# Cheng-Lin-Li/show-attend-and-tell

Hardware: AMD Instinct MI355X
Metric: training images/sec (higher is better)
Workload: dtype bf16; 1 GPU; model=vgg16_frozen+attention_lstm512, global_batch=32, seq_len=20, vocab=5000, parallelism=dp1

## Files before the change

sat_amd/models/bptt.py:

```python

import torch

from sat_amd import _C

ACT_NONE, ACT_TANH, ACT_RELU = 0, 1, 2


def _drop(x, seed, p, salt):
    if p <= 0.0:
        return x
    return _C.hash_dropout(x, seed, p, salt)


class DecoderCoreBPTT(torch.autograd.Function):

    @staticmethod
    def forward(ctx_ag, contexts, init_memory, init_output, sentences,
                masks, emb, w1a, b1a, w1b, b1b, v, wl, bl, seed,
                p_fc, p_lstm, train_cnn, shadows=None):
        if shadows is not None:
            emb_c = shadows['emb']
            w1a_c, b1a_c = shadows['w1a'], shadows['b1a']
            w1b_c, b1b_c = shadows['w1b'], shadows['b1b']
            v_c = shadows['v'].reshape(-1)
            wl_c, bl_c = shadows['wl'], shadows['bl']
        else:
            emb_c, w1a_c, b1a_c = emb, w1a, b1a
            w1b_c, b1b_c, v_c = w1b, b1b, v
            wl_c, bl_c = wl, bl
        B, L, D = contexts.shape
        T = sentences.shape[1]
        A = w1a_c.shape[0]
        H = init_memory.shape[1]
        E = emb_c.shape[1]
        I = D + E
        dev = contexts.device

        ctx_flat = contexts.reshape(B * L, D)
        if p_fc > 0.0:
            CDROP = _C.hash_dropout_steps(ctx_flat, seed, p_fc, 0, 16, T)
            T1 = _C.dense_fwd(CDROP.reshape(T * B * L, D), w1a_c,
                              b1a_c, 1)
        else:
            CDROP = None
            T1 = _C.dense_fwd(ctx_flat, w1a_c, b1a_c, 1)

        XH = torch.empty(T * B, I + H, dtype=torch.bfloat16, device=dev)
        EXPD = torch.empty(T * B, H + D + E, dtype=torch.bfloat16,
                           device=dev)
        ODROP = torch.empty(T * B, H, dtype=torch.bfloat16, device=dev)

        t1s, t2s, tdrops, alphas = [], [], [], []
        gates_l, cprev_l = [], []

        labels_cat = sentences.t().reshape(-1)

        memory = init_memory
        state_h = init_output
        last_word = torch.zeros(B, dtype=torch.int64, device=dev)
        empty_b = _EMPTY_B(dev)
        fuse_small = (B <= 128 and (I + H) % 32 == 0
                      and (H + D + E) % 32 == 0)

        _C.hash_dropout_out(init_output, seed, p_fc, 1, ODROP[0:B])

        for t in range(T):
            s = t * 16
            sl = slice(t * B, (t + 1) * B)

            t1 = T1.reshape(-1, A)[t * B * L:(t + 1) * B * L] \
                if CDROP is not None else T1
            t2 = _C.dense_fwd(ODROP[sl], w1b_c, b1b_c, ACT_TANH)
            tdrop, att_logits = _C.attn_scores_fused(
                t1, t2, v_c, seed, p_fc, s + 2, L)
            alpha, pooled = _C.attn_pool_fwd(contexts, att_logits)

            _C.lstm_in_fuse(pooled, emb_c, last_word, state_h, seed,
                            p_lstm, s + 3, XH[sl])
            od_next = ODROP[(t + 1) * B:(t + 2) * B] if t + 1 < T \
                else empty_b
            if fuse_small:
                gates, c_new, sth_t = _C.dense_lstm_expand_fwd(
                    XH[sl], wl_c, bl_c, memory, pooled, emb_c,
                    last_word, seed, EXPD[sl], od_next,
                    1.0, p_lstm, p_fc, s)
            else:
                gates = _C.dense_fwd(XH[sl], wl_c, bl_c, ACT_NONE)
                h_raw, c_new = _C.lstm_pointwise_fwd(gates, memory, 1.0)
                out_t, sth_t = _C.expand_fuse(
                    h_raw, pooled, emb_c, last_word, seed, EXPD[sl],
                    od_next, p_lstm, p_fc, s)

            t1s.append(t1)
            t2s.append(t2)
            tdrops.append(tdrop)
            alphas.append(alpha)
            gates_l.append(gates)
            cprev_l.append(memory)

            memory = c_new
            state_h = sth_t
            last_word = labels_cat[sl]

        alpha_stack = torch.stack(alphas)
        attn_acc = (alpha_stack
                    * masks.t().reshape(T, B, 1)).sum(dim=0)

        ctx_ag.save_for_backward(
            contexts, emb_c, w1a_c, b1a_c, w1b_c, b1b_c, v_c, wl_c,
            bl_c, seed, XH, ODROP, labels_cat, masks)
        ctx_ag.leaf_mode = shadows is not None
        ctx_ag.cdrop = CDROP
        ctx_ag.saved_lists = (t1s, t2s, tdrops, alphas, gates_l, cprev_l)
        ctx_ag.dims = (B, L, D, T, A, H, E, I)
        ctx_ag.p_fc = p_fc
        ctx_ag.p_lstm = p_lstm
        ctx_ag.train_cnn = train_cnn
        return EXPD, attn_acc

    @staticmethod
    def backward(ctx_ag, d_expd, d_attn):
        (contexts, emb, w1a, b1a, w1b, b1b, v, wl, bl, seed, XH,
         ODROP, labels_cat, masks) = ctx_ag.saved_tensors
        (t1s, t2s, tdrops, alphas, gates_l,
         cprev_l) = ctx_ag.saved_lists
        B, L, D, T, A, H, E, I = ctx_ag.dims
        p_fc = ctx_ag.p_fc
        p_lstm = ctx_ag.p_lstm
        dev = contexts.device
        need_dctx = ctx_ag.train_cnn and ctx_ag.needs_input_grad[0]

        ctx_flat = contexts.reshape(B * L, D)
        if not d_expd.is_contiguous():
            d_expd = d_expd.contiguous()

        wl_t = wl.t().contiguous()
        w1b_t = w1b.t().contiguous()

        DG = torch.empty(T * B, 4 * H, dtype=torch.bfloat16, device=dev)
        DEMB = torch.empty(T * B, E, dtype=torch.bfloat16, device=dev)
        DPRE1B = torch.empty(T * B, A, dtype=torch.bfloat16, device=dev)
        DPRE1A = torch.empty(T * B * L, A, dtype=torch.bfloat16,
                             device=dev)
        CDROP = ctx_ag.cdrop

        dv_acc = torch.zeros_like(v, dtype=torch.float32)
        dctx_acc = torch.zeros_like(contexts) if need_dctx else None

        d_out_carry = torch.zeros(B, H, dtype=torch.bfloat16, device=dev)
        d_sth_carry = torch.zeros(B, H, dtype=torch.bfloat16, device=dev)
        dc_carry = torch.zeros(B, H, dtype=torch.bfloat16, device=dev)

        for t in range(T - 1, -1, -1):
            s = t * 16
            sl = slice(t * B, (t + 1) * B)
            dc_prev, dpool_dec, demb_dec = _C.dexp_lstm_bwd(
                d_expd[sl], d_out_carry, d_sth_carry, seed,
                gates_l[t], cprev_l[t], dc_carry, DG[sl],
                p_fc, p_lstm, s, D, E, 1.0)
            dgates = DG[sl]
            if B <= 128:
                dpooled, d_sth_carry = _C.dense_dx_fuse(
                    dgates, wl_t, dpool_dec, demb_dec, seed, DEMB[sl],
                    p_lstm, s + 3, D, E, H)
            else:
                dxh = _C.dense_fwd(dgates, wl_t, _EMPTY_B(dev),
                                   ACT_NONE)
                dpooled, d_sth_carry = _C.dx_fuse(
                    dxh, dpool_dec, demb_dec, seed, DEMB[sl], p_lstm,
                    s + 3, H)
            dc_carry = dc_prev

            dalpha_t = d_attn * masks[:, t].unsqueeze(1)
            dlog_att, dctx_t = _C.attn_pool_bwd(
                contexts, alphas[t], dalpha_t.contiguous(),
                dpooled, need_dctx)
            if need_dctx:
                dctx_acc += dctx_t
            sl_a = slice(t * B * L, (t + 1) * B * L)
            _dt1, dt2f, _dv = _C.attn_scores_bwd_tanh(
                tdrops[t], v, dlog_att, seed, p_fc, s + 2, L, dv_acc,
                t1s[t], DPRE1A[sl_a])

            _C.act_bwd_f32_out(dt2f, t2s[t], ACT_TANH, DPRE1B[sl])
            d_out_carry = _C.dense_fwd_drop(DPRE1B[sl], w1b_t, seed,
                                            p_fc, s + 1)

            if need_dctx:
                dcd = DPRE1A[sl_a].matmul(w1a)
                dctx_acc += _drop(dcd, seed, p_fc, s + 0) \
                    .reshape(B, L, D)

        if CDROP is not None:
            dW1a = torch.bmm(
                DPRE1A.reshape(T, B * L, A).transpose(1, 2),
                CDROP.reshape(T, B * L, D)).sum(dim=0)
        else:
            dW1a = DPRE1A.reshape(T, B * L, A).sum(0).t() \
                .matmul(ctx_flat)
        db1a = DPRE1A.sum(0, dtype=torch.float32)
        dWl = DG.t().matmul(XH)
        dbl = DG.sum(0, dtype=torch.float32)
        dW1b = DPRE1B.t().matmul(ODROP)
        db1b = DPRE1B.sum(0, dtype=torch.float32)
        demb_table = _C.embedding_bwd(
            torch.cat([torch.zeros(B, dtype=torch.int64, device=dev),
                       labels_cat[:-B]]),
            DEMB, emb.shape[0])

        d_init_output = (d_out_carry.float()
                         + d_sth_carry.float()).to(torch.bfloat16)
        d_init_memory = dc_carry

        if ctx_ag.leaf_mode:
            return (dctx_acc, d_init_memory, d_init_output, None, None,
                    demb_table.float(), dW1a.float(), db1a,
                    dW1b.float(), db1b, dv_acc.reshape(1, -1),
                    dWl.float(), dbl, None, None, None, None, None)
        bf = torch.bfloat16
        return (dctx_acc, d_init_memory, d_init_output, None, None,
                demb_table.to(bf), dW1a.to(bf), db1a.to(bf),
                dW1b.to(bf), db1b.to(bf), dv_acc.to(bf),
                dWl.to(bf), dbl.to(bf), None, None, None, None, None)


class DecodeHeadBPTT(torch.autograd.Function):

    @staticmethod
    def forward(ctx_ag, expd, wd1, bd1, wd2, bd2, sentences, masks,
                seed, p_fc, shadows=None):
        B, T = sentences.shape
        V = wd2.shape[0]
        bf = torch.bfloat16

        if shadows is not None:
            wd1c, bd1c = shadows['wd1'], shadows['bd1']
            wd2c, bd2c = shadows['wd2'], shadows['bd2']
        else:
            wd1c = wd1.to(bf)
            bd1c = bd1.to(bf)
            wd2c = wd2.to(bf)
            bd2c = bd2.to(bf)

        HID = _C.dense_fwd(expd, wd1c, bd1c, ACT_TANH)
        HD = _C.hash_dropout_slabs(HID, seed, p_fc, 7, 16, T) \
            if p_fc > 0.0 else HID
        LOGITS = _C.dense_fwd(HD, wd2c, bd2c, ACT_NONE)

        labels_cat = sentences.t().reshape(-1)
        masks_cat = masks.t().reshape(-1).contiguous()
        CE, LSE = _C.ce_fwd(LOGITS, labels_cat, masks_cat)
        ce = CE.reshape(T, B).t().contiguous()
        predictions = LOGITS.reshape(T, B, V).argmax(dim=2) \
            .t().contiguous()

        ctx_ag.save_for_backward(expd, wd1c, wd2c, HID, HD, LOGITS,
                                 LSE, labels_cat, masks_cat, seed)
        ctx_ag.T = T
        ctx_ag.p_fc = p_fc
        ctx_ag.mark_non_differentiable(predictions)
        return ce, predictions

    @staticmethod
    def backward(ctx_ag, d_ce, _d_pred):
        (expd, wd1c, wd2c, HID, HD, LOGITS, LSE, labels_cat,
         masks_cat, seed) = ctx_ag.saved_tensors
        T = ctx_ag.T
        p_fc = ctx_ag.p_fc

        dce_cat = d_ce.t().reshape(-1).contiguous().float()
        DL = _C.ce_bwd(LOGITS, labels_cat, masks_cat, LSE, dce_cat)

        fast_dx = wd2c.shape[0] % 8 == 0 and wd1c.shape[0] % 8 == 0
        if fast_dx:
            wd2_t = wd2c.t().contiguous()
            wd1_t = wd1c.t().contiguous()
            eb = torch.empty(0, dtype=torch.bfloat16, device=DL.device)
            DHD = _C.dense_fwd(DL, wd2_t, eb, 0)
        else:
            DHD = DL.matmul(wd2c)
        DHID = _C.hash_dropout_slabs(DHD, seed, p_fc, 7, 16, T) \
            if p_fc > 0.0 else DHD
        DP1 = _C.act_bwd(DHID, HID, ACT_TANH)

        if fast_dx and DL.shape[0] % 8 == 0:
            dWd2 = _C.dense_fwd(DL.t().contiguous(),
                                HD.t().contiguous(), eb, 0).float()
        else:
            dWd2 = DL.t().matmul(HD).float()
        dbd2 = DL.sum(0, dtype=torch.float32)
        dWd1 = DP1.t().matmul(expd).float()
        dbd1 = DP1.sum(0, dtype=torch.float32)
        d_expd = _C.dense_fwd(DP1, wd1_t, eb, 0) if fast_dx \
            else DP1.matmul(wd1c)

        return (d_expd, dWd1, dbd1, dWd2, dbd2, None, None, None, None,
                None)


_EMPTY = {}


def _EMPTY_B(device):
    key = str(device)
    if key not in _EMPTY:
        _EMPTY[key] = torch.empty(0, device=device, dtype=torch.bfloat16)
    return _EMPTY[key]


def run_decoder_bptt(decoder, contexts, init_memory, init_output,
                     sentences, masks):
    d = decoder
    sh = getattr(d, '_shadows', None) \
        if getattr(d, '_shadows_active', False) else None
    if sh:
        expd, attn_acc = DecoderCoreBPTT.apply(
            contexts, init_memory, init_output, sentences, masks,
            d.embedding, d.att_fc_1a.weight, d.att_fc_1a.bias,
            d.att_fc_1b.weight, d.att_fc_1b.bias, d.att_fc_2.weight,
            d.lstm_w, d.lstm_b,
            d._rng, d.nn.fc_drop_rate, d.nn.lstm_drop_rate,
            d.nn.train_cnn, sh)
        ce, predictions = DecodeHeadBPTT.apply(
            expd, d.dec_fc_1.weight, d.dec_fc_1.bias,
            d.dec_fc_2.weight, d.dec_fc_2.bias,
            sentences, masks, d._rng, d.nn.fc_drop_rate, sh)
        return ce, attn_acc, predictions
    expd, attn_acc = DecoderCoreBPTT.apply(
        contexts, init_memory, init_output, sentences, masks,
        d._emb_c, d.att_fc_1a._wc, d.att_fc_1a._bc,
        d.att_fc_1b._wc, d.att_fc_1b._bc, d._att_vc,
        d._lstm_wc, d._lstm_bc,
        d._rng, d.nn.fc_drop_rate, d.nn.lstm_drop_rate,
        d.nn.train_cnn, None)
    ce, predictions = DecodeHeadBPTT.apply(
        expd, d.dec_fc_1.weight, d.dec_fc_1.bias,
        d.dec_fc_2.weight, d.dec_fc_2.bias,
        sentences, masks, d._rng, d.nn.fc_drop_rate, None)
    return ce, attn_acc, predictions
```

sat_amd/ops/csrc/bindings.cpp:

```cpp
#include <torch/extension.h>
#include <vector>

at::Tensor dense_fwd(at::Tensor x, at::Tensor w, at::Tensor bias, int64_t act);
at::Tensor dense_fwd_drop(at::Tensor x, at::Tensor w, at::Tensor seed,
                          double p, int64_t salt);
std::vector<at::Tensor> dense_lstm_expand_fwd(
        at::Tensor xh, at::Tensor wl, at::Tensor bl, at::Tensor c_prev,
        at::Tensor pooled, at::Tensor table, at::Tensor ids,
        at::Tensor seed, at::Tensor expdrop, at::Tensor od_next,
        double fb, double p_lstm, double p_fc, int64_t s);
std::vector<at::Tensor> dexp_lstm_bwd(at::Tensor dexpd,
                                      at::Tensor d_out_carry,
                                      at::Tensor d_sth_carry,
                                      at::Tensor seed, at::Tensor gates,
                                      at::Tensor c_prev, at::Tensor dc,
                                      at::Tensor dgates_out,
                                      double p_fc, double p_lstm,
                                      int64_t s, int64_t D, int64_t E,
                                      double fb);
std::vector<at::Tensor> dense_dx_fuse(at::Tensor dgates, at::Tensor wl_t,
                                      at::Tensor dpool_dec,
                                      at::Tensor demb_dec,
                                      at::Tensor seed,
                                      at::Tensor demb_out,
                                      double p, int64_t salt,
                                      int64_t D, int64_t E, int64_t H);
at::Tensor conv3_fwd(at::Tensor input, at::Tensor weight, at::Tensor bias,
                     bool relu, bool emit_pad);
void bias_act_nhwc(at::Tensor y, at::Tensor bias, bool relu);
void scale_bias_act_nhwc(at::Tensor y, at::Tensor scale, at::Tensor shift,
                         bool relu);
at::Tensor maxpool2x2_nhwc(at::Tensor input);
at::Tensor conv_igemm_fwd(at::Tensor input, at::Tensor w_ohwi,
                          at::Tensor bias, bool relu);
at::Tensor pad1_nhwc(at::Tensor input);
at::Tensor conv_igemm_8p_fwd(at::Tensor padded, at::Tensor w_ohwi,
                             at::Tensor bias, int64_t Hh, int64_t Ww,
                             bool relu);
at::Tensor conv_igemm_glds64_fwd(at::Tensor padded, at::Tensor w_ohwi,
                                 at::Tensor bias, int64_t Hh, int64_t Ww,
                                 bool relu);
at::Tensor dense_8p_fwd(at::Tensor x, at::Tensor w, at::Tensor bias,
                        int64_t act);
at::Tensor conv3x3_wgrad(at::Tensor xpad, at::Tensor dy_rows,
                         int64_t Hh, int64_t Ww);
at::Tensor conv_igemm_glds_fwd(at::Tensor padded, at::Tensor w_ohwi,
                               at::Tensor bias, int64_t Hh, int64_t Ww,
                               bool relu);
std::vector<at::Tensor> dense_lstm_fwd(at::Tensor xh, at::Tensor wl,
                                       at::Tensor bl, at::Tensor c_prev,
                                       double fb);
std::vector<at::Tensor> lstm_pointwise_bwd_out(at::Tensor gates,
                                               at::Tensor c, at::Tensor dh,
                                               at::Tensor dc, double fb,
                                               at::Tensor dgates_out);
void lstm_in_fuse(at::Tensor pooled, at::Tensor table, at::Tensor ids,
                  at::Tensor sth, at::Tensor seed, double p, int64_t salt,
                  at::Tensor xh);
std::vector<at::Tensor> expand_fuse(at::Tensor h_raw, at::Tensor pooled,
                                    at::Tensor table, at::Tensor ids,
                                    at::Tensor seed,
                                    at::Tensor expdrop, at::Tensor od_next,
                                    double p_lstm, double p_fc, int64_t s);
std::vector<at::Tensor> dexp_fuse(at::Tensor dexpd, at::Tensor d_out_carry,
                                  at::Tensor d_sth_carry, at::Tensor seed,
                                  double p_fc, double p_lstm, int64_t s,
                                  int64_t D, int64_t E);
std::vector<at::Tensor> dx_fuse(at::Tensor dxh, at::Tensor dpool_dec,
                                at::Tensor demb_dec, at::Tensor seed,
                                at::Tensor demb_out, double p,
                                int64_t salt, int64_t H);
void hash_dropout_out(at::Tensor x, at::Tensor seed, double p,
                      int64_t salt, at::Tensor out);
at::Tensor hash_dropout_steps(at::Tensor x, at::Tensor seed, double p,
                              int64_t salt_base, int64_t salt_stride,
                              int64_t T);
void act_bwd_out(at::Tensor dy, at::Tensor y, int64_t act, at::Tensor out);
at::Tensor hash_dropout_slabs(at::Tensor x, at::Tensor seed, double p,
                              int64_t salt_base, int64_t salt_stride,
                              int64_t T);
std::vector<at::Tensor> lstm_pointwise_fwd(at::Tensor gates, at::Tensor c,
                                           double fb);
std::vector<at::Tensor> lstm_pointwise_bwd(at::Tensor gates, at::Tensor c,
                                           at::Tensor dh, at::Tensor dc,
                                           double fb);
at::Tensor act_bwd(at::Tensor dy, at::Tensor y, int64_t act);
void act_bwd_f32_out(at::Tensor dy, at::Tensor y, int64_t act,
                     at::Tensor out);
at::Tensor hash_dropout(at::Tensor x, at::Tensor seed, double p,
                        int64_t salt);
std::vector<at::Tensor> attn_pool_fwd(at::Tensor ctx, at::Tensor logits);
std::vector<at::Tensor> attn_scores_fused(at::Tensor t1, at::Tensor t2,
                                          at::Tensor v, at::Tensor seed,
                                          double p, int64_t salt, int64_t L);
std::vector<at::Tensor> attn_pool_bwd(at::Tensor ctx, at::Tensor alpha,
                                      at::Tensor dalpha, at::Tensor dpooled,
                                      bool need_dctx);
std::vector<at::Tensor> attn_scores_bwd(at::Tensor tdrop, at::Tensor v,
                                        at::Tensor dlogits, at::Tensor seed,
                                        double p, int64_t salt, int64_t L);
std::vector<at::Tensor> attn_scores_bwd_acc(at::Tensor tdrop, at::Tensor v,
                                            at::Tensor dlogits,
                                            at::Tensor seed, double p,
                                            int64_t salt, int64_t L,
                                            at::Tensor dv_acc);
std::vector<at::Tensor> attn_scores_bwd_tanh(
        at::Tensor tdrop, at::Tensor v, at::Tensor dlogits,
        at::Tensor seed, double p, int64_t salt, int64_t L,
        at::Tensor dv_acc, at::Tensor t1y, at::Tensor dt1_out);
at::Tensor embedding_fwd(at::Tensor ids, at::Tensor table);
at::Tensor embedding_bwd(at::Tensor ids, at::Tensor dy, int64_t rows);
std::vector<at::Tensor> ce_fwd(at::Tensor logits, at::Tensor labels,
                               at::Tensor mask);
at::Tensor ce_bwd(at::Tensor logits, at::Tensor labels, at::Tensor mask,
                  at::Tensor lse, at::Tensor dloss);
at::Tensor grad_sq_norm(std::vector<at::Tensor> grads);
at::Tensor sq_norm_mt(at::Tensor desc, at::Tensor cum, int64_t n_tensors,
                      int64_t total);
void adam_step_mt(at::Tensor desc, at::Tensor cum, int64_t n_tensors,
                  int64_t total, at::Tensor step_dev, double lr0,
                  double decay_factor, double steps_per_decay, double b1,
                  double b2, double eps, double clip, at::Tensor gsq,
                  bool zero_grads, bool vec4);
void adam_step(std::vector<at::Tensor> params, std::vector<at::Tensor> grads,
               std::vector<at::Tensor> ms, std::vector<at::Tensor> vs,
               at::Tensor step_dev, double lr0, double decay_factor,
               double steps_per_decay, double b1, double b2, double eps,
               double clip, at::Tensor gsq);

PYBIND11_MODULE(TORCH_EXTENSION_NAME, m) {
    m.def("dense_fwd", &dense_fwd, "MFMA GEMM + bias/act (bf16)");
    m.def("dense_fwd_drop", &dense_fwd_drop,
          "skinny GEMM with hash-dropout fused into the split-K epilogue");
    m.def("dense_lstm_expand_fwd", &dense_lstm_expand_fwd,
          "gates GEMM + LSTM gate math + expand scatter in 2 launches");
    m.def("dexp_lstm_bwd", &dexp_lstm_bwd,
          "dexp scatter + LSTM pointwise backward in one launch");
    m.def("dense_dx_fuse", &dense_dx_fuse,
          "dxh GEMM with the dx scatter fused into the epilogue");
    m.def("bias_act_nhwc", &bias_act_nhwc);
    m.def("scale_bias_act_nhwc", &scale_bias_act_nhwc);
    m.def("maxpool2x2_nhwc", &maxpool2x2_nhwc);
    m.def("conv_igemm_fwd", &conv_igemm_fwd);
    m.def("pad1_nhwc", &pad1_nhwc);
    m.def("conv_igemm_glds_fwd", &conv_igemm_glds_fwd);
    m.def("conv_igemm_8p_fwd", &conv_igemm_8p_fwd,
          "8-phase deep-pipelined implicit-GEMM conv (Cout%256==0)");
    m.def("conv_igemm_glds64_fwd", &conv_igemm_glds64_fwd);
    m.def("dense_8p_fwd", &dense_8p_fwd,
          "8-phase deep-pipelined dense GEMM (big-M shapes)");
    m.def("conv3x3_wgrad", &conv3x3_wgrad,
          "3x3 conv weight grad: transpose-staged MFMA split-K reduce");
    m.def("dense_lstm_fwd", &dense_lstm_fwd);
    m.def("conv3_fwd", &conv3_fwd,
          "direct NHWC conv for 3-channel 3x3/s1 (VGG conv1_1)");
    m.def("lstm_pointwise_bwd_out", &lstm_pointwise_bwd_out);
    m.def("lstm_in_fuse", &lstm_in_fuse);
    m.def("expand_fuse", &expand_fuse);
    m.def("dexp_fuse", &dexp_fuse);
    m.def("dx_fuse", &dx_fuse);
    m.def("hash_dropout_out", &hash_dropout_out);
    m.def("hash_dropout_steps", &hash_dropout_steps);
    m.def("act_bwd_out", &act_bwd_out);
    m.def("hash_dropout_slabs", &hash_dropout_slabs);
    m.def("lstm_pointwise_fwd", &lstm_pointwise_fwd);
    m.def("lstm_pointwise_bwd", &lstm_pointwise_bwd);
    m.def("act_bwd", &act_bwd);
    m.def("act_bwd_f32_out", &act_bwd_f32_out);
    m.def("hash_dropout", &hash_dropout);
    m.def("attn_pool_fwd", &attn_pool_fwd);
    m.def("attn_scores_fused", &attn_scores_fused);
    m.def("attn_pool_bwd", &attn_pool_bwd);
    m.def("attn_scores_bwd", &attn_scores_bwd);
    m.def("attn_scores_bwd_acc", &attn_scores_bwd_acc);
    m.def("attn_scores_bwd_tanh", &attn_scores_bwd_tanh,
          "scores backward with fused tanh-bwd dt1 into a given slab");
    m.def("embedding_fwd", &embedding_fwd);
    m.def("embedding_bwd", &embedding_bwd);
    m.def("ce_fwd", &ce_fwd);
    m.def("ce_bwd", &ce_bwd);
    m.def("grad_sq_norm", &grad_sq_norm);
    m.def("sq_norm_mt", &sq_norm_mt);
    m.def("adam_step_mt", &adam_step_mt);
    m.def("adam_step", &adam_step);
}
```

sat_amd/ops/csrc/bptt_fuse.hip:

```cpp

#include "common.h"


__global__ void lstm_in_fuse_kernel(const bf16* __restrict__ pooled,
                                    const bf16* __restrict__ table,
                                    const int64_t* __restrict__ ids,
                                    const bf16* __restrict__ sth,
                                    const int64_t* __restrict__ seed_p,
                                    bf16* __restrict__ xh,
                                    int B, int D, int E, int H,
                                    float p, int salt) {
    const uint32_t seed = (uint32_t)(*seed_p);
    const int I = D + E;
    const int W = I + H;
    int64_t idx = (int64_t)blockIdx.x * blockDim.x + threadIdx.x;
    if (idx >= (int64_t)B * W) return;
    int b = idx / W, j = idx % W;
    float val;
    if (j < I) {
        val = (j < D) ? bf2f(pooled[(int64_t)b * D + j])
                      : bf2f(table[ids[b] * E + (j - D)]);
        val *= drop_scale(seed, salt, (uint32_t)(b * I + j), p);
    } else {
        val = bf2f(sth[(int64_t)b * H + (j - I)]);
    }
    xh[idx] = f2bf(val);
}

void lstm_in_fuse(at::Tensor pooled, at::Tensor table, at::Tensor ids,
                  at::Tensor sth, at::Tensor seed, double p, int64_t salt,
                  at::Tensor xh) {
    int B = pooled.size(0), D = pooled.size(1), E = table.size(1),
        H = sth.size(1);
    int64_t n = (int64_t)B * (D + E + H);
    hipStream_t s = at::cuda::getCurrentCUDAStream();
    hipLaunchKernelGGL(lstm_in_fuse_kernel, dim3(cdiv(n, 256)), dim3(256),
                       0, s,
                       (const bf16*)pooled.data_ptr(),
                       (const bf16*)table.data_ptr(),
                       (const int64_t*)ids.data_ptr(),
                       (const bf16*)sth.data_ptr(),
                       (const int64_t*)seed.data_ptr(),
                       (bf16*)xh.data_ptr(), B, D, E, H,
                       (float)p, (int)salt);
    HIP_OK(hipGetLastError());
}


__global__ void expand_fuse_kernel(const bf16* __restrict__ h_raw,
                                   const bf16* __restrict__ pooled,
                                   const bf16* __restrict__ table,
                                   const int64_t* __restrict__ ids,
                                   const int64_t* __restrict__ seed_p,
                                   bf16* __restrict__ out_t,
                                   bf16* __restrict__ sth_t,
                                   bf16* __restrict__ expdrop,
                                   bf16* __restrict__ od_next,
                                   int B, int H, int D, int E,
                                   float p_lstm, float p_fc, int s) {
    const uint32_t seed = (uint32_t)(*seed_p);
    const int W = H + D + E;
    int64_t idx = (int64_t)blockIdx.x * blockDim.x + threadIdx.x;
    if (idx >= (int64_t)B * W) return;
    int b = idx / W, j = idx % W;
    float val;
    if (j < H) {
        float h = bf2f(h_raw[(int64_t)b * H + j]);
        uint32_t hidx = (uint32_t)(b * H + j);
        float ot = h * drop_scale(seed, s + 4, hidx, p_lstm);
        out_t[(int64_t)b * H + j] = f2bf(ot);
        sth_t[(int64_t)b * H + j] =
            f2bf(h * drop_scale(seed, s + 5, hidx, p_lstm));
        if (od_next != nullptr)
            od_next[(int64_t)b * H + j] =
                f2bf(ot * drop_scale(seed, s + 16 + 1, hidx, p_fc));
        val = ot;
    } else if (j < H + D) {
        val = bf2f(pooled[(int64_t)b * D + (j - H)]);
    } else {
        val = bf2f(table[ids[b] * E + (j - H - D)]);
    }
    expdrop[idx] = f2bf(val * drop_scale(seed, s + 6,
                                         (uint32_t)(b * W + j), p_fc));
}

std::vector<at::Tensor> expand_fuse(at::Tensor h_raw, at::Tensor pooled,
                                    at::Tensor table, at::Tensor ids,
                                    at::Tensor seed,
                                    at::Tensor expdrop, at::Tensor od_next,
                                    double p_lstm, double p_fc,
                                    int64_t s) {
    int B = h_raw.size(0), H = h_raw.size(1), D = pooled.size(1),
        E = table.size(1);
    auto out_t = at::empty_like(h_raw);
    auto sth_t = at::empty_like(h_raw);
    bf16* od_ptr = nullptr;
    if (od_next.defined() && od_next.numel() > 0)
        od_ptr = (bf16*)od_next.data_ptr();
    int64_t n = (int64_t)B * (H + D + E);
    hipStream_t st = at::cuda::getCurrentCUDAStream();
    hipLaunchKernelGGL(expand_fuse_kernel, dim3(cdiv(n, 256)), dim3(256),
                       0, st,
                       (const bf16*)h_raw.data_ptr(),
                       (const bf16*)pooled.data_ptr(),
                       (const bf16*)table.data_ptr(),
                       (const int64_t*)ids.data_ptr(),
                       (const int64_t*)seed.data_ptr(),
                       (bf16*)out_t.data_ptr(), (bf16*)sth_t.data_ptr(),
                       (bf16*)expdrop.data_ptr(), od_ptr,
                       B, H, D, E, (float)p_lstm, (float)p_fc, (int)s);
    HIP_OK(hipGetLastError());
    return {out_t, sth_t};
}


__global__ void dexp_fuse_kernel(const bf16* __restrict__ dexpd,
                                 const bf16* __restrict__ d_out_carry,
                                 const bf16* __restrict__ d_sth_carry,
                                 const int64_t* __restrict__ seed_p,
                                 bf16* __restrict__ dh_raw,
                                 bf16* __restrict__ dpool_dec,
                                 bf16* __restrict__ demb_dec,
                                 int B, int H, int D, int E,
                                 float p_fc, float p_lstm, int s) {
    const uint32_t seed = (uint32_t)(*seed_p);
    const int W = H + D + E;
    int64_t idx = (int64_t)blockIdx.x * blockDim.x + threadIdx.x;
    if (idx >= (int64_t)B * W) return;
    int b = idx / W, j = idx % W;
    float dexp = bf2f(dexpd[idx])
        * drop_scale(seed, s + 6, (uint32_t)(b * W + j), p_fc);
    if (j < H) {
        uint32_t hidx = (uint32_t)(b * H + j);
        float dout = dexp + bf2f(d_out_carry[(int64_t)b * H + j]);
        float dh = dout * drop_scale(seed, s + 4, hidx, p_lstm)
            + bf2f(d_sth_carry[(int64_t)b * H + j])
            * drop_scale(seed, s + 5, hidx, p_lstm);
        dh_raw[(int64_t)b * H + j] = f2bf(dh);
    } else if (j < H + D) {
        dpool_dec[(int64_t)b * D + (j - H)] = f2bf(dexp);
    } else {
        demb_dec[(int64_t)b * E + (j - H - D)] = f2bf(dexp);
    }
}

std::vector<at::Tensor> dexp_fuse(at::Tensor dexpd, at::Tensor d_out_carry,
                                  at::Tensor d_sth_carry, at::Tensor seed,
                                  double p_fc, double p_lstm, int64_t s,
                                  int64_t D, int64_t E) {
    int B = d_out_carry.size(0), H = d_out_carry.size(1);
    auto dh_raw = at::empty_like(d_out_carry);
    auto dpool = at::empty({B, D}, d_out_carry.options());
    auto demb = at::empty({B, E}, d_out_carry.options());
    int64_t n = (int64_t)B * (H + D + E);
    hipStream_t st = at::cuda::getCurrentCUDAStream();
    hipLaunchKernelGGL(dexp_fuse_kernel, dim3(cdiv(n, 256)), dim3(256),
                       0, st,
                       (const bf16*)dexpd.data_ptr(),
                       (const bf16*)d_out_carry.data_ptr(),
                       (const bf16*)d_sth_carry.data_ptr(),
                       (const int64_t*)seed.data_ptr(),
                       (bf16*)dh_raw.data_ptr(), (bf16*)dpool.data_ptr(),
                       (bf16*)demb.data_ptr(), B, H, (int)D, (int)E,
                       (float)p_fc, (float)p_lstm, (int)s);
    HIP_OK(hipGetLastError());
    return {dh_raw, dpool, demb};
}


__global__ void dx_fuse_kernel(const bf16* __restrict__ dxh,
                               const bf16* __restrict__ dpool_dec,
                               const bf16* __restrict__ demb_dec,
                               const int64_t* __restrict__ seed_p,
                               bf16* __restrict__ dpooled,
                               bf16* __restrict__ demb_out,
                               bf16* __restrict__ dsth,
                               int B, int D, int E, int H,
                               float p, int salt) {
    const uint32_t seed = (uint32_t)(*seed_p);
    const int I = D + E;
    const int W = I + H;
    int64_t idx = (int64_t)blockIdx.x * blockDim.x + threadIdx.x;
    if (idx >= (int64_t)B * W) return;
    int b = idx / W, j = idx % W;
    float g = bf2f(dxh[idx]);
    if (j < I) {
        g *= drop_scale(seed, salt, (uint32_t)(b * I + j), p);
        if (j < D)
            dpooled[(int64_t)b * D + j] =
                f2bf(g + bf2f(dpool_dec[(int64_t)b * D + j]));
        else
            demb_out[(int64_t)b * E + (j - D)] =
                f2bf(g + bf2f(demb_dec[(int64_t)b * E + (j - D)]));
    } else {
        dsth[(int64_t)b * H + (j - I)] = f2bf(g);
    }
}

std::vector<at::Tensor> dx_fuse(at::Tensor dxh, at::Tensor dpool_dec,
                                at::Tensor demb_dec, at::Tensor seed,
                                at::Tensor demb_out, double p,
                                int64_t salt, int64_t H) {
    int B = dpool_dec.size(0), D = dpool_dec.size(1), E = demb_dec.size(1);
    auto dpooled = at::empty_like(dpool_dec);
    auto dsth = at::empty({B, H}, dpool_dec.options());
    int64_t n = (int64_t)B * (D + E + H);
    hipStream_t st = at::cuda::getCurrentCUDAStream();
    hipLaunchKernelGGL(dx_fuse_kernel, dim3(cdiv(n, 256)), dim3(256),
                       0, st,
                       (const bf16*)dxh.data_ptr(),
                       (const bf16*)dpool_dec.data_ptr(),
                       (const bf16*)demb_dec.data_ptr(),
                       (const int64_t*)seed.data_ptr(),
                       (bf16*)dpooled.data_ptr(),
                       (bf16*)demb_out.data_ptr(),
                       (bf16*)dsth.data_ptr(),
                       B, D, E, (int)H, (float)p, (int)salt);
    HIP_OK(hipGetLastError());
    return {dpooled, dsth};
}


__global__ void hash_dropout_out_kernel(const bf16* __restrict__ x,
                                        const int64_t* __restrict__ seed_p,
                                        bf16* __restrict__ y,
                                        int64_t n, float p, int salt) {
    const uint32_t seed = (uint32_t)(*seed_p);
    int64_t idx = (int64_t)blockIdx.x * blockDim.x + threadIdx.x;
    if (idx >= n) return;
    y[idx] = f2bf(bf2f(x[idx])
                  * drop_scale(seed, salt, (uint32_t)idx, p));
}

void hash_dropout_out(at::Tensor x, at::Tensor seed, double p,
                      int64_t salt, at::Tensor out) {
    int64_t n = x.numel();
    hipStream_t s = at::cuda::getCurrentCUDAStream();
    hipLaunchKernelGGL(hash_dropout_out_kernel, dim3(cdiv(n, 256)),
                       dim3(256), 0, s,
                       (const bf16*)x.data_ptr(),
                       (const int64_t*)seed.data_ptr(),
                       (bf16*)out.data_ptr(), n, (float)p, (int)salt);
    HIP_OK(hipGetLastError());
}


__global__ void hash_dropout_steps_kernel(const bf16* __restrict__ x,
                                          const int64_t* __restrict__ seed_p,
                                          bf16* __restrict__ y,
                                          int64_t n, int T, float p,
                                          int salt_base, int salt_stride) {
    const uint32_t seed = (uint32_t)(*seed_p);
    int64_t i8 = ((int64_t)blockIdx.x * blockDim.x + threadIdx.x) * 8;
    int64_t total = n * T;
    int64_t stride = (int64_t)gridDim.x * blockDim.x * 8;
    for (; i8 < total; i8 += stride) {
        int t = (int)(i8 / n);
        int64_t j = i8 % n;
        int salt = salt_base + t * salt_stride;
        bf16x8 v = *(const bf16x8*)(x + j);
        bf16x8 o;
#pragma unroll
        for (int e = 0; e < 8; ++e)
            o[e] = f2bf(bf2f(v[e]) * drop_scale(seed, salt,
                                                (uint32_t)(j + e), p));
        *(bf16x8*)(y + i8) = o;
    }
}

at::Tensor hash_dropout_steps(at::Tensor x, at::Tensor seed, double p,
                              int64_t salt_base, int64_t salt_stride,
                              int64_t T) {
    int64_t n = x.numel();
    TORCH_CHECK(n % 8 == 0, "hash_dropout_steps needs numel % 8 == 0");
    auto y = at::empty({T, x.size(0), x.size(1)}, x.options());
    hipStream_t s = at::cuda::getCurrentCUDAStream();
    int blocks = (int)std::min<int64_t>(cdiv(n * T, 256 * 8), 16384);
    hipLaunchKernelGGL(hash_dropout_steps_kernel, dim3(blocks), dim3(256),
                       0, s,
                       (const bf16*)x.data_ptr(),
                       (const int64_t*)seed.data_ptr(),
                       (bf16*)y.data_ptr(), n, (int)T, (float)p,
                       (int)salt_base, (int)salt_stride);
    HIP_OK(hipGetLastError());
    return y;
}

__global__ void act_bwd_out_kernel(const bf16* __restrict__ dy,
                                   const bf16* __restrict__ y,
                                   bf16* __restrict__ dpre,
                                   int64_t n, int act) {
    int64_t idx = (int64_t)blockIdx.x * blockDim.x + threadIdx.x;
    if (idx >= n) return;
    float g = bf2f(dy[idx]);
    float yv = bf2f(y[idx]);
    if (act == 1) g *= (1.f - yv * yv);
    else if (act == 2) g *= (yv > 0.f ? 1.f : 0.f);
    dpre[idx] = f2bf(g);
}

void act_bwd_out(at::Tensor dy, at::Tensor y, int64_t act, at::Tensor out) {
    int64_t n = dy.numel();
    hipStream_t s = at::cuda::getCurrentCUDAStream();
    hipLaunchKernelGGL(act_bwd_out_kernel, dim3(cdiv(n, 256)), dim3(256),
                       0, s,
                       (const bf16*)dy.data_ptr(), (const bf16*)y.data_ptr(),
                       (bf16*)out.data_ptr(), n, (int)act);
    HIP_OK(hipGetLastError());
}

__global__ void act_bwd_f32_out_kernel(const float* __restrict__ dy,
                                       const bf16* __restrict__ y,
                                       bf16* __restrict__ dpre,
                                       int64_t n, int act) {
    int64_t idx = (int64_t)blockIdx.x * blockDim.x + threadIdx.x;
    if (idx >= n) return;
    float g = dy[idx];
    float yv = bf2f(y[idx]);
    if (act == 1) g *= (1.f - yv * yv);
    else if (act == 2) g *= (yv > 0.f ? 1.f : 0.f);
    dpre[idx] = f2bf(g);
}

void act_bwd_f32_out(at::Tensor dy, at::Tensor y, int64_t act,
                     at::Tensor out) {
    int64_t n = dy.numel();
    hipStream_t s = at::cuda::getCurrentCUDAStream();
    hipLaunchKernelGGL(act_bwd_f32_out_kernel, dim3(cdiv(n, 256)),
                       dim3(256), 0, s,
                       (const float*)dy.data_ptr(),
                       (const bf16*)y.data_ptr(),
                       (bf16*)out.data_ptr(), n, (int)act);
    HIP_OK(hipGetLastError());
}


__global__ void hash_dropout_slabs_kernel(const bf16* __restrict__ x,
                                          const int64_t* __restrict__ seed_p,
                                          bf16* __restrict__ y,
                                          int64_t slab_elems, int T,
                                          float p, int salt_base,
                                          int salt_stride) {
    const uint32_t seed = (uint32_t)(*seed_p);
    int64_t i8 = ((int64_t)blockIdx.x * blockDim.x + threadIdx.x) * 8;
    int64_t total = slab_elems * T;
    if (i8 >= total) return;
    int t = (int)(i8 / slab_elems);
    int64_t j = i8 % slab_elems;
    int salt = salt_base + t * salt_stride;
    bf16x8 v = *(const bf16x8*)(x + i8);
    bf16x8 o;
#pragma unroll
    for (int e = 0; e < 8; ++e)
        o[e] = f2bf(bf2f(v[e])
                    * drop_scale(seed, salt, (uint32_t)(j + e), p));
    *(bf16x8*)(y + i8) = o;
}

at::Tensor hash_dropout_slabs(at::Tensor x, at::Tensor seed, double p,
                              int64_t salt_base, int64_t salt_stride,
                              int64_t T) {
    if (p <= 0.0) return x;
    int64_t n = x.numel();
    int64_t slab = n / T;
    TORCH_CHECK(slab % 8 == 0 && n % T == 0);
    auto y = at::empty_like(x);
    hipStream_t s = at::cuda::getCurrentCUDAStream();
    hipLaunchKernelGGL(hash_dropout_slabs_kernel,
                       dim3(cdiv(n / 8, 256)), dim3(256), 0, s,
                       (const bf16*)x.data_ptr(),
                       (const int64_t*)seed.data_ptr(),
                       (bf16*)y.data_ptr(), slab, (int)T, (float)p,
                       (int)salt_base, (int)salt_stride);
    HIP_OK(hipGetLastError());
    return y;
}


__global__ void dexp_lstm_bwd_kernel(const bf16* __restrict__ dexpd,
                                     const bf16* __restrict__ d_out_carry,
                                     const bf16* __restrict__ d_sth_carry,
                                     const int64_t* __restrict__ seed_p,
                                     const bf16* __restrict__ gates,
                                     const bf16* __restrict__ c,
                                     const bf16* __restrict__ dc,
                                     bf16* __restrict__ dgates,
                                     bf16* __restrict__ dc_prev,
                                     bf16* __restrict__ dpool_dec,
                                     bf16* __restrict__ demb_dec,
                                     int B, int H, int D, int E,
                                     float p_fc, float p_lstm, int s,
                                     float fb) {
    const uint32_t seed = (uint32_t)(*seed_p);
    const int W = H + D + E;
    int64_t idx = (int64_t)blockIdx.x * blockDim.x + threadIdx.x;
    if (idx >= (int64_t)B * W) return;
    int b = idx / W, j = idx % W;
    float dexp = bf2f(dexpd[idx])
        * drop_scale(seed, s + 6, (uint32_t)(b * W + j), p_fc);
    if (j < H) {
        uint32_t hidx = (uint32_t)(b * H + j);
        float dout = dexp + bf2f(d_out_carry[(int64_t)b * H + j]);
        float dhv = dout * drop_scale(seed, s + 4, hidx, p_lstm)
            + bf2f(d_sth_carry[(int64_t)b * H + j])
            * drop_scale(seed, s + 5, hidx, p_lstm);
        const bf16* gp = gates + (int64_t)b * 4 * H + j;
        float g[4], dg[4], dcp;
#pragma unroll
        for (int q = 0; q < 4; ++q) g[q] = bf2f(gp[q * H]);
        float dcv = (dc != nullptr) ? bf2f(dc[(int64_t)b * H + j]) : 0.f;
        lstm_cell_bwd(g, bf2f(c[(int64_t)b * H + j]), dhv, dcv, fb, dg,
                      dcp);
        bf16* dgp = dgates + (int64_t)b * 4 * H + j;
#pragma unroll
        for (int q = 0; q < 4; ++q) dgp[q * H] = f2bf(dg[q]);
        dc_prev[(int64_t)b * H + j] = f2bf(dcp);
    } else if (j < H + D) {
        dpool_dec[(int64_t)b * D + (j - H)] = f2bf(dexp);
    } else {
        demb_dec[(int64_t)b * E + (j - H - D)] = f2bf(dexp);
    }
}

std::vector<at::Tensor> dexp_lstm_bwd(at::Tensor dexpd,
                                      at::Tensor d_out_carry,
                                      at::Tensor d_sth_carry,
                                      at::Tensor seed, at::Tensor gates,
                                      at::Tensor c_prev, at::Tensor dc,
                                      at::Tensor dgates_out,
                                      double p_fc, double p_lstm,
                                      int64_t s, int64_t D, int64_t E,
                                      double fb) {
    CHECK_GPU(dexpd); CHECK_BF16(dexpd);
    int B = d_out_carry.size(0), H = d_out_carry.size(1);
    TORCH_CHECK(dexpd.numel() == (int64_t)B * (H + D + E));
    TORCH_CHECK(dgates_out.numel() == (int64_t)B * 4 * H);
    auto dc_prev = at::empty({B, H}, dexpd.options());
    auto dpool_dec = at::empty({B, D}, dexpd.options());
    auto demb_dec = at::empty({B, E}, dexpd.options());
    const bf16* dc_ptr = nullptr;
    if (dc.defined() && dc.numel() > 0)
        dc_ptr = (const bf16*)dc.data_ptr();
    int64_t n = (int64_t)B * (H + D + E);
    hipStream_t st = at::cuda::getCurrentCUDAStream();
    hipLaunchKernelGGL(dexp_lstm_bwd_kernel, dim3(cdiv(n, 256)),
                       dim3(256), 0, st,
                       (const bf16*)dexpd.data_ptr(),
                       (const bf16*)d_out_carry.data_ptr(),
                       (const bf16*)d_sth_carry.data_ptr(),
                       (const int64_t*)seed.data_ptr(),
                       (const bf16*)gates.data_ptr(),
                       (const bf16*)c_prev.data_ptr(), dc_ptr,
                       (bf16*)dgates_out.data_ptr(),
                       (bf16*)dc_prev.data_ptr(),
                       (bf16*)dpool_dec.data_ptr(),
                       (bf16*)demb_dec.data_ptr(),
                       B, H, (int)D, (int)E,
                       (float)p_fc, (float)p_lstm, (int)s, (float)fb);
    HIP_OK(hipGetLastError());
    return {dc_prev, dpool_dec, demb_dec};
}
```

sat_amd/ops/csrc/gemm.hip:

```cpp

#include "common.h"

at::Tensor dense_8p_fwd(at::Tensor x, at::Tensor w, at::Tensor bias,
                        int64_t act);
at::Tensor hash_dropout(at::Tensor x, at::Tensor seed, double p,
                        int64_t salt);

#define BK 64
#define LDS_STRIDE (BK + 8)

#define ACT_NONE 0
#define ACT_TANH 1
#define ACT_RELU 2

__device__ __forceinline__ float apply_act(float v, int act) {
    if (act == ACT_TANH) return tanhf(v);
    if (act == ACT_RELU) return fmaxf(v, 0.f);
    return v;
}


template <int WR, int WC, int FM, int FN>
__global__ __launch_bounds__(256)
void tiled_gemm_kernel(const bf16* __restrict__ A,
                       const bf16* __restrict__ W,
                       const bf16* __restrict__ bias,
                       bf16* __restrict__ Y,
                       int M, int N, int K, int act,
                       float* __restrict__ Yf, int kchunk) {
    constexpr int BM = WR * FM * 16;
    constexpr int BN = WC * FN * 16;
    __shared__ bf16 As[BM * LDS_STRIDE];
    __shared__ bf16 Bs[BN * LDS_STRIDE];

    const int tid = threadIdx.x;
    const int lane = tid & 63;
    const int wave = tid >> 6;
    const int wr = wave / WC;
    const int wc = wave % WC;

    const int bm = blockIdx.y * BM;
    const int bn = blockIdx.x * BN;

    floatx4 acc[FM][FN];
#pragma unroll
    for (int i = 0; i < FM; ++i)
#pragma unroll
        for (int j = 0; j < FN; ++j)
            acc[i][j] = floatx4{0.f, 0.f, 0.f, 0.f};

    const int lrow = lane & 15;
    const int kgrp = lane >> 4;

    constexpr int A_CHUNKS = BM * BK / 8 / 256;
    constexpr int B_CHUNKS = BN * BK / 8 / 256;

    int kbeg = 0, kend = K;
    if (Yf != nullptr) {
        kbeg = blockIdx.z * kchunk;
        kend = min(K, kbeg + kchunk);
    }
    for (int k0 = kbeg; k0 < kend; k0 += BK) {
#pragma unroll
        for (int i = 0; i < A_CHUNKS; ++i) {
            int q = tid + 256 * i;
            int row = q >> 3;
            int c8 = (q & 7) * 8;
            int gk = k0 + c8;
            bf16x8 v = {};
            int ga = bm + row;
            if (ga < M && gk + 8 <= K) {
                v = *(const bf16x8*)(A + (int64_t)ga * K + gk);
            } else if (ga < M) {
                for (int e = 0; e < 8; ++e)
                    if (gk + e < K) v[e] = A[(int64_t)ga * K + gk + e];
            }
            *(bf16x8*)(As + row * LDS_STRIDE + c8) = v;
        }
#pragma unroll
        for (int i = 0; i < B_CHUNKS; ++i) {
            int q = tid + 256 * i;
            int row = q >> 3;
            int c8 = (q & 7) * 8;
            int gk = k0 + c8;
            bf16x8 v = {};
            int gb = bn + row;
            if (gb < N && gk + 8 <= K) {
                v = *(const bf16x8*)(W + (int64_t)gb * K + gk);
            } else if (gb < N) {
                for (int e = 0; e < 8; ++e)
                    if (gk + e < K) v[e] = W[(int64_t)gb * K + gk + e];
            }
            *(bf16x8*)(Bs + row * LDS_STRIDE + c8) = v;
        }
        __syncthreads();

#pragma unroll
        for (int kk = 0; kk < BK / 32; ++kk) {
            bf16x8 a_frag[FM], b_frag[FN];
            const int kof = kk * 32 + kgrp * 8;
#pragma unroll
            for (int mi = 0; mi < FM; ++mi)
                a_frag[mi] = *(const bf16x8*)(
                    As + (wr * FM * 16 + mi * 16 + lrow) * LDS_STRIDE + kof);
#pragma unroll
            for (int ni = 0; ni < FN; ++ni)
                b_frag[ni] = *(const bf16x8*)(
                    Bs + (wc * FN * 16 + ni * 16 + lrow) * LDS_STRIDE + kof);
#pragma unroll
            for (int mi = 0; mi < FM; ++mi)
#pragma unroll
                for (int ni = 0; ni < FN; ++ni)
                    acc[mi][ni] = __builtin_amdgcn_mfma_f32_16x16x32_bf16(
                        a_frag[mi], b_frag[ni], acc[mi][ni], 0, 0, 0);
        }
        __syncthreads();
    }

    float* slab = (Yf != nullptr)
        ? Yf + (int64_t)blockIdx.z * M * N : nullptr;
#pragma unroll
    for (int ni = 0; ni < FN; ++ni) {
        int col = bn + wc * FN * 16 + ni * 16 + (lane & 15);
        float bv = (bias != nullptr && col < N) ? bf2f(bias[col]) : 0.f;
#pragma unroll
        for (int mi = 0; mi < FM; ++mi) {
#pragma unroll
            for (int r = 0; r < 4; ++r) {
                int row = bm + wr * FM * 16 + mi * 16 + (lane >> 4) * 4 + r;
                if (row < M && col < N) {
                    if (slab != nullptr)
                        slab[(int64_t)row * N + col] = acc[mi][ni][r];
                    else
                        Y[(int64_t)row * N + col] =
                            f2bf(apply_act(acc[mi][ni][r] + bv, act));
                }
            }
        }
    }
}


template <int RF>
__global__ __launch_bounds__(256)
void skinny_gemm_kernel(const bf16* __restrict__ A,
                        const bf16* __restrict__ W,
                        const bf16* __restrict__ bias,
                        bf16* __restrict__ Y,
                        float* __restrict__ Yf,
                        int M, int N, int K, int act, int splitk) {
    const int lane = threadIdx.x & 63;
    const int wave = threadIdx.x >> 6;
    const int n0 = blockIdx.x * 64 + wave * 16;
    const bool active = (n0 < N);

    const int kq = blockIdx.y;
    const int kchunk = ((K / 32 + splitk - 1) / splitk) * 32;
    const int kbeg = kq * kchunk;
    const int kend = min(K, kbeg + kchunk);

    const int lrow = lane & 15;
    const int kgrp = lane >> 4;

    floatx4 acc[RF];
#pragma unroll
    for (int i = 0; i < RF; ++i)
        acc[i] = floatx4{0.f, 0.f, 0.f, 0.f};

    const bool wfull = (n0 + 16 <= N);
    if (active) {
        for (int k = kbeg; k < kend; k += 32) {
            const int kof = k + kgrp * 8;
            bf16x8 b_frag = {};
            if (kof + 8 <= K) {
                int gb = n0 + lrow;
                if (wfull || gb < N)
                    b_frag = *(const bf16x8*)(W + (int64_t)gb * K + kof);
            } else if (kof < K) {
                int gb = n0 + lrow;
                if (wfull || gb < N)
                    for (int e = 0; e < 8 && kof + e < K; ++e)
                        b_frag[e] = W[(int64_t)gb * K + kof + e];
            }
#pragma unroll
            for (int mi = 0; mi < RF; ++mi) {
                bf16x8 a0 = {};
                int ar = mi * 16 + lrow;
                if (kof + 8 <= K) {
                    if (ar < M)
                        a0 = *(const bf16x8*)(A + (int64_t)ar * K + kof);
                } else if (kof < K) {
                    if (ar < M)
                        for (int e = 0; e < 8 && kof + e < K; ++e)
                            a0[e] = A[(int64_t)ar * K + kof + e];
                }
                acc[mi] = __builtin_amdgcn_mfma_f32_16x16x32_bf16(
                    a0, b_frag, acc[mi], 0, 0, 0);
            }
        }
    }

    const int col = n0 + (lane & 15);
    if (!active || col >= N) return;
    if (Yf == nullptr) {
        float bv = (bias != nullptr) ? bf2f(bias[col]) : 0.f;
#pragma unroll
        for (int mi = 0; mi < RF; ++mi)
#pragma unroll
            for (int r = 0; r < 4; ++r) {
                int row = mi * 16 + (lane >> 4) * 4 + r;
                if (row < M)
                    Y[(int64_t)row * N + col] =
                        f2bf(apply_act(acc[mi][r] + bv, act));
            }
        return;
    }

    float* slab = Yf + (int64_t)kq * M * N;
#pragma unroll
    for (int mi = 0; mi < RF; ++mi)
#pragma unroll
        for (int r = 0; r < 4; ++r) {
            int row = mi * 16 + (lane >> 4) * 4 + r;
            if (row < M)
                slab[(int64_t)row * N + col] = acc[mi][r];
        }
}

__global__ void skinny_epilogue_kernel(const float* __restrict__ Yf,
                                       const bf16* __restrict__ bias,
                                       bf16* __restrict__ Y,
                                       int64_t n, int N, int act,
                                       int splitk) {
    int64_t idx = (int64_t)blockIdx.x * blockDim.x + threadIdx.x;
    if (idx >= n) return;
    float v = sum_slabs(Yf, n, idx, splitk);
    if (bias != nullptr) v += bf2f(bias[idx % N]);
    Y[idx] = f2bf(apply_act(v, act));
}

__global__ void dense_glds_kernel(const bf16* __restrict__ A,
                                  const bf16* __restrict__ W,
                                  const bf16* __restrict__ bias,
                                  bf16* __restrict__ Y,
                                  int M, int N, int K, int act);


static bool is_skinny(int64_t M, int64_t K) {
    return M <= 128 && K % 32 == 0;
}

struct SkinnyPlan { int nblocks, splitk; };

static SkinnyPlan skinny_plan(int64_t N, int64_t K) {
    int nblocks = cdiv(N, 64);
    int splitk = 1;
    while (nblocks * splitk < 192 && splitk < 8 &&
           (int)(K / 32) >= 2 * splitk)
        splitk *= 2;
    return {nblocks, splitk};
}

static void launch_skinny(hipStream_t stream, const at::Tensor& x,
                          const at::Tensor& w, const bf16* bias, bf16* y,
                          float* yf, int act, SkinnyPlan plan) {
    const int M = x.size(0), K = x.size(1), N = w.size(0);
    TORCH_CHECK(is_skinny(M, K),
                "skinny GEMM: M <= 128 and K % 32 == 0 only");
    auto kernel = M <= 32 ? skinny_gemm_kernel<2>
                : M <= 64 ? skinny_gemm_kernel<4>
                          : skinny_gemm_kernel<8>;
    hipLaunchKernelGGL(kernel, dim3(plan.nblocks, plan.splitk), dim3(256),
                       0, stream, (const bf16*)x.data_ptr(),
                       (const bf16*)w.data_ptr(), bias, y, yf, M, N, K,
                       act, plan.splitk);
}

static at::Tensor skinny_slabs(hipStream_t stream, const at::Tensor& x,
                               const at::Tensor& w) {
    SkinnyPlan plan = skinny_plan(w.size(0), x.size(1));
    auto yf = at::empty({plan.splitk, x.size(0), w.size(0)},
                        x.options().dtype(at::kFloat));
    launch_skinny(stream, x, w, nullptr, nullptr, (float*)yf.data_ptr(),
                  ACT_NONE, plan);
    return yf;
}

static void launch_tiled(hipStream_t stream, const at::Tensor& x,
                         const at::Tensor& w, const bf16* bias, bf16* y,
                         float* yf, int act, int splitk, int kchunk) {
    const int M = x.size(0), K = x.size(1), N = w.size(0);
    const bool narrow = N <= 512;
    auto kernel = narrow ? tiled_gemm_kernel<4, 1, 2, 4>
                         : tiled_gemm_kernel<2, 2, 4, 4>;
    dim3 grid(cdiv(N, narrow ? 64 : 128), cdiv(M, 128), splitk);
    hipLaunchKernelGGL(kernel, grid, dim3(256), 0, stream,
                       (const bf16*)x.data_ptr(),
                       (const bf16*)w.data_ptr(), bias, y, M, N, K, act,
                       yf, kchunk);
}

static void launch_epilogue(hipStream_t stream, const at::Tensor& yf,
                            const bf16* bias, at::Tensor& y, int act) {
    int64_t n = y.numel();
    hipLaunchKernelGGL(skinny_epilogue_kernel, dim3(cdiv(n, 256)),
                       dim3(256), 0, stream, (const float*)yf.data_ptr(),
                       bias, (bf16*)y.data_ptr(), n, (int)y.size(1), act,
                       (int)yf.size(0));
}

at::Tensor dense_fwd(at::Tensor x, at::Tensor w, at::Tensor bias,
                     int64_t act) {
    CHECK_GPU(x); CHECK_CONTIG(x); CHECK_BF16(x);
    CHECK_GPU(w); CHECK_CONTIG(w); CHECK_BF16(w);
    TORCH_CHECK(x.dim() == 2 && w.dim() == 2, "dense_fwd expects 2-D inputs");
    const int64_t M = x.size(0), K = x.size(1), N = w.size(0);
    TORCH_CHECK(w.size(1) == K, "weight inner dim mismatch");
    TORCH_CHECK(K % 8 == 0, "K must be a multiple of 8 (bf16x8 loads)");
    const bf16* bias_ptr = nullptr;
    if (bias.defined() && bias.numel() > 0) {
        CHECK_GPU(bias); CHECK_CONTIG(bias); CHECK_BF16(bias);
        TORCH_CHECK(bias.numel() == N, "bias size mismatch");
        bias_ptr = (const bf16*)bias.data_ptr();
    }
    const bool skinny = is_skinny(M, K);
    if (!skinny && M >= 16384 && N >= 256 && N % 8 == 0 && K % 64 == 0
        && K >= 128) {
        return dense_8p_fwd(x, w, bias_ptr != nullptr ? bias : at::Tensor(),
                            act);
    }
    auto y = at::empty({M, N}, x.options());
    hipStream_t stream = at::cuda::getCurrentCUDAStream();

    if (skinny) {
        SkinnyPlan plan = skinny_plan(N, K);
        if (plan.splitk == 1) {
            launch_skinny(stream, x, w, bias_ptr, (bf16*)y.data_ptr(),
                          nullptr, (int)act, plan);
        } else {
            auto yf = skinny_slabs(stream, x, w);
            launch_epilogue(stream, yf, bias_ptr, y, (int)act);
        }
    } else if (M >= 16384 && N % 128 == 0 && K % 64 == 0) {
        dim3 grid(cdiv(N, 128), cdiv(M, 128));
        hipLaunchKernelGGL(dense_glds_kernel, grid, dim3(256), 0,
                           stream,
                           (const bf16*)x.data_ptr(),
                           (const bf16*)w.data_ptr(), bias_ptr,
                           (bf16*)y.data_ptr(), (int)M, (int)N, (int)K,
                           (int)act);
    } else {
        int tiles = cdiv(N, N <= 512 ? 64 : 128) * cdiv(M, 128);
        int splitk = 1;
        while (tiles * splitk < 160 && splitk < 8
               && K >= 128 * 2 * splitk)
            splitk *= 2;
        int kchunk = cdiv(cdiv(K, splitk), 64) * 64;
        splitk = cdiv(K, kchunk);
        if (splitk == 1) {
            launch_tiled(stream, x, w, bias_ptr, (bf16*)y.data_ptr(),
                         nullptr, (int)act, 1, kchunk);
        } else {
            auto yf = at::empty({splitk, M, N},
                                x.options().dtype(at::kFloat));
            launch_tiled(stream, x, w, bias_ptr, (bf16*)y.data_ptr(),
                         (float*)yf.data_ptr(), (int)act, splitk, kchunk);
            launch_epilogue(stream, yf, bias_ptr, y, (int)act);
        }
    }
    HIP_OK(hipGetLastError());
    return y;
}


__global__ void skinny_epilogue_drop_kernel(
        const float* __restrict__ Yf, bf16* __restrict__ Y,
        const int64_t* __restrict__ seed_p, int64_t n, int splitk,
        float p, int salt) {
    int64_t idx = (int64_t)blockIdx.x * blockDim.x + threadIdx.x;
    if (idx >= n) return;
    float v = sum_slabs(Yf, n, idx, splitk);
    v *= drop_scale((uint32_t)(*seed_p), salt, (uint32_t)idx, p);
    Y[idx] = f2bf(v);
}

at::Tensor dense_fwd_drop(at::Tensor x, at::Tensor w, at::Tensor seed,
                          double p, int64_t salt) {
    CHECK_GPU(x); CHECK_CONTIG(x); CHECK_BF16(x);
    CHECK_GPU(w); CHECK_CONTIG(w); CHECK_BF16(w);
    int64_t M = x.size(0), K = x.size(1), N = w.size(0);
    if (p <= 0.0 || !is_skinny(M, K)) {
        auto y = dense_fwd(x, w, at::Tensor(), ACT_NONE);
        return p > 0.0 ? hash_dropout(y, seed, p, salt) : y;
    }
    auto y = at::empty({M, N}, x.options());
    hipStream_t stream = at::cuda::getCurrentCUDAStream();
    auto yf = skinny_slabs(stream, x, w);
    int64_t n = M * N;
    hipLaunchKernelGGL(skinny_epilogue_drop_kernel,
                       dim3(cdiv(n, 256)), dim3(256), 0, stream,
                       (const float*)yf.data_ptr(), (bf16*)y.data_ptr(),
                       (const int64_t*)seed.data_ptr(), n,
                       (int)yf.size(0), (float)p, (int)salt);
    HIP_OK(hipGetLastError());
    return y;
}


__device__ __forceinline__ void sum_gates(const float* __restrict__ Yf,
                                          const bf16* __restrict__ bias,
                                          bf16* __restrict__ gates,
                                          int B, int H, int b, int hh,
                                          int splitk, float g[4]) {
    int64_t n = (int64_t)B * 4 * H;
#pragma unroll
    for (int q = 0; q < 4; ++q) {
        int64_t off = (int64_t)b * 4 * H + q * H + hh;
        float acc = sum_slabs(Yf, n, off, splitk);
        if (bias != nullptr) acc += bf2f(bias[q * H + hh]);
        gates[off] = f2bf(acc);
        g[q] = acc;
    }
}

__global__ void skinny_epi_lstm_kernel(const float* __restrict__ Yf,
                                       const bf16* __restrict__ bias,
                                       const bf16* __restrict__ c_prev,
                                       bf16* __restrict__ gates,
                                       bf16* __restrict__ h_out,
                                       bf16* __restrict__ c_out,
                                       int B, int H, int splitk,
                                       float fb) {
    int idx = blockIdx.x * blockDim.x + threadIdx.x;
    if (idx >= B * H) return;
    float g[4], cn, h;
    sum_gates(Yf, bias, gates, B, H, idx / H, idx % H, splitk, g);
    lstm_cell_fwd(g, bf2f(c_prev[idx]), fb, cn, h);
    h_out[idx] = f2bf(h);
    c_out[idx] = f2bf(cn);
}

std::vector<at::Tensor> dense_lstm_fwd(at::Tensor xh, at::Tensor wl,
                                       at::Tensor bl, at::Tensor c_prev,
                                       double fb) {
    int64_t M = xh.size(0), N = wl.size(0);
    int B = c_prev.size(0), H = c_prev.size(1);
    TORCH_CHECK(M == B && N == 4 * H);
    auto gates = at::empty({M, N}, xh.options());
    auto h_out = at::empty_like(c_prev);
    auto c_out = at::empty_like(c_prev);
    hipStream_t s = at::cuda::getCurrentCUDAStream();
    auto yf = skinny_slabs(s, xh, wl);
    hipLaunchKernelGGL(skinny_epi_lstm_kernel,
                       dim3(cdiv(B * H, 256)), dim3(256), 0, s,
                       (const float*)yf.data_ptr(),
                       (const bf16*)bl.data_ptr(),
                       (const bf16*)c_prev.data_ptr(),
                       (bf16*)gates.data_ptr(), (bf16*)h_out.data_ptr(),
                       (bf16*)c_out.data_ptr(), B, H, (int)yf.size(0),
                       (float)fb);
    HIP_OK(hipGetLastError());
    return {gates, h_out, c_out};
}



__global__ __launch_bounds__(256)
void dense_glds_kernel(const bf16* __restrict__ A,
                       const bf16* __restrict__ W,
                       const bf16* __restrict__ bias,
                       bf16* __restrict__ Y,
                       int M, int N, int K, int act) {
    constexpr int BM = 128, BN = 128, BKc = 64;
    __shared__ bf16 lds[2 * BM * BKc];
    bf16* As = lds;
    bf16* Bs = lds + BM * BKc;

    const int tid = threadIdx.x;
    const int lane = tid & 63;
    const int wave = tid >> 6;
    const int wr = wave >> 1, wc = wave & 1;
    const int bm = blockIdx.y * BM;
    const int bn = blockIdx.x * BN;

    const bf16* aSrc[4];
    const bf16* wSrc[4];
    const int ci8 = (lane & 7) * 8;
#pragma unroll
    for (int i = 0; i < 4; ++i) {
        int r = wave * 32 + i * 8 + (lane >> 3);
        int swz = (r & 4) ? 16 : 0;
        int ga = bm + r;
        if (ga >= M) ga = M - 1;
        aSrc[i] = A + (int64_t)ga * K + (ci8 ^ swz);
        int gb = bn + r;
        if (gb >= N) gb = N - 1;
        wSrc[i] = W + (int64_t)gb * K + (ci8 ^ swz);
    }

    floatx4 acc[4][4];
#pragma unroll
    for (int i = 0; i < 4; ++i)
#pragma unroll
        for (int j = 0; j < 4; ++j)
            acc[i][j] = floatx4{0.f, 0.f, 0.f, 0.f};

    const int lrow = lane & 15;
    const int kgrp = lane >> 4;

    for (int k0 = 0; k0 < K; k0 += BKc) {
#pragma unroll
        for (int i = 0; i < 4; ++i) {
            __builtin_amdgcn_global_load_lds(
                (const __attribute__((address_space(1))) uint32_t*)
                    (aSrc[i] + k0),
                (__attribute__((address_space(3))) uint32_t*)
                    (As + (wave * 32 + i * 8) * BKc),
                16, 0, 0);
            __builtin_amdgcn_global_load_lds(
                (const __attribute__((address_space(1))) uint32_t*)
                    (wSrc[i] + k0),
                (__attribute__((address_space(3))) uint32_t*)
                    (Bs + (wave * 32 + i * 8) * BKc),
                16, 0, 0);
        }
        __syncthreads();

#pragma unroll
        for (int kk = 0; kk < 2; ++kk) {
            bf16x8 a_frag[4], b_frag[4];
            const int kof = kk * 32 + kgrp * 8;
#pragma unroll
            for (int mi = 0; mi < 4; ++mi) {
                int r = wr * 64 + mi * 16 + lrow;
                a_frag[mi] = *(const bf16x8*)(
                    As + r * BKc + (kof ^ ((r & 4) ? 16 : 0)));
            }
#pragma unroll
            for (int ni = 0; ni < 4; ++ni) {
                int r = wc * 64 + ni * 16 + lrow;
                b_frag[ni] = *(const bf16x8*)(
                    Bs + r * BKc + (kof ^ ((r & 4) ? 16 : 0)));
            }
#pragma unroll
            for (int mi = 0; mi < 4; ++mi)
#pragma unroll
                for (int ni = 0; ni < 4; ++ni)
                    acc[mi][ni] = __builtin_amdgcn_mfma_f32_16x16x32_bf16(
                        a_frag[mi], b_frag[ni], acc[mi][ni], 0, 0, 0);
        }
        __syncthreads();
    }

#pragma unroll
    for (int ni = 0; ni < 4; ++ni) {
        int col = bn + wc * 64 + ni * 16 + (lane & 15);
        float bv = (bias != nullptr && col < N) ? bf2f(bias[col]) : 0.f;
#pragma unroll
        for (int mi = 0; mi < 4; ++mi) {
#pragma unroll
            for (int r = 0; r < 4; ++r) {
                int row = bm + wr * 64 + mi * 16 + (lane >> 4) * 4 + r;
                if (row < M && col < N) {
                    float vv = acc[mi][ni][r] + bv;
                    Y[(int64_t)row * N + col] = f2bf(apply_act(vv, act));
                }
            }
        }
    }
}


__global__ void skinny_epi_dx_kernel(const float* __restrict__ Yf,
                                     const bf16* __restrict__ dpool_dec,
                                     const bf16* __restrict__ demb_dec,
                                     const int64_t* __restrict__ seed_p,
                                     bf16* __restrict__ dpooled,
                                     bf16* __restrict__ demb_out,
                                     bf16* __restrict__ dsth,
                                     int64_t n, int splitk,
                                     int B, int D, int E, int H,
                                     float p, int salt) {
    const uint32_t seed = (uint32_t)(*seed_p);
    const int I = D + E;
    const int W = I + H;
    int64_t idx = (int64_t)blockIdx.x * blockDim.x + threadIdx.x;
    if (idx >= n) return;
    float g = sum_slabs(Yf, n, idx, splitk);
    int b = (int)(idx / W), j = (int)(idx % W);
    if (j < I) {
        g *= drop_scale(seed, salt, (uint32_t)(b * I + j), p);
        if (j < D)
            dpooled[(int64_t)b * D + j] =
                f2bf(g + bf2f(dpool_dec[(int64_t)b * D + j]));
        else
            demb_out[(int64_t)b * E + (j - D)] =
                f2bf(g + bf2f(demb_dec[(int64_t)b * E + (j - D)]));
    } else {
        dsth[(int64_t)b * H + (j - I)] = f2bf(g);
    }
}

std::vector<at::Tensor> dense_dx_fuse(at::Tensor dgates, at::Tensor wl_t,
                                      at::Tensor dpool_dec,
                                      at::Tensor demb_dec,
                                      at::Tensor seed,
                                      at::Tensor demb_out,
                                      double p, int64_t salt,
                                      int64_t D, int64_t E, int64_t H) {
    CHECK_GPU(dgates); CHECK_CONTIG(dgates); CHECK_BF16(dgates);
    CHECK_GPU(wl_t); CHECK_CONTIG(wl_t); CHECK_BF16(wl_t);
    int64_t M = dgates.size(0), N = wl_t.size(0);
    TORCH_CHECK(N == D + E + H);
    auto dpooled = at::empty({M, D}, dgates.options());
    auto dsth = at::empty({M, H}, dgates.options());
    hipStream_t stream = at::cuda::getCurrentCUDAStream();
    auto yf = skinny_slabs(stream, dgates, wl_t);
    int64_t n = M * N;
    hipLaunchKernelGGL(skinny_epi_dx_kernel, dim3(cdiv(n, 256)),
                       dim3(256), 0, stream,
                       (const float*)yf.data_ptr(),
                       (const bf16*)dpool_dec.data_ptr(),
                       (const bf16*)demb_dec.data_ptr(),
                       (const int64_t*)seed.data_ptr(),
                       (bf16*)dpooled.data_ptr(),
                       (bf16*)demb_out.data_ptr(),
                       (bf16*)dsth.data_ptr(),
                       n, (int)yf.size(0), (int)M, (int)D, (int)E, (int)H,
                       (float)p, (int)salt);
    HIP_OK(hipGetLastError());
    return {dpooled, dsth};
}


__global__ void skinny_epi_lstm_expand_kernel(
        const float* __restrict__ Yf, const bf16* __restrict__ bias,
        const bf16* __restrict__ c_prev,
        const bf16* __restrict__ pooled,
        const bf16* __restrict__ table,
        const int64_t* __restrict__ ids,
        const int64_t* __restrict__ seed_p,
        bf16* __restrict__ gates, bf16* __restrict__ c_out,
        bf16* __restrict__ sth_t, bf16* __restrict__ expdrop,
        bf16* __restrict__ od_next,
        int B, int H, int D, int E, int splitk,
        float fb, float p_lstm, float p_fc, int s) {
    const uint32_t seed = (uint32_t)(*seed_p);
    const int W = H + D + E;
    int64_t idx = (int64_t)blockIdx.x * blockDim.x + threadIdx.x;
    if (idx >= (int64_t)B * W) return;
    int b = idx / W, j = idx % W;
    float val;
    if (j < H) {
        float g[4], cn, h;
        sum_gates(Yf, bias, gates, B, H, b, j, splitk, g);
        lstm_cell_fwd(g, bf2f(c_prev[(int64_t)b * H + j]), fb, cn, h);
        c_out[(int64_t)b * H + j] = f2bf(cn);
        uint32_t hidx = (uint32_t)(b * H + j);
        float ot = h * drop_scale(seed, s + 4, hidx, p_lstm);
        sth_t[(int64_t)b * H + j] =
            f2bf(h * drop_scale(seed, s + 5, hidx, p_lstm));
        if (od_next != nullptr)
            od_next[(int64_t)b * H + j] =
                f2bf(ot * drop_scale(seed, s + 16 + 1, hidx, p_fc));
        val = ot;
    } else if (j < H + D) {
        val = bf2f(pooled[(int64_t)b * D + (j - H)]);
    } else {
        val = bf2f(table[ids[b] * E + (j - H - D)]);
    }
    expdrop[idx] = f2bf(val * drop_scale(seed, s + 6,
                                         (uint32_t)(b * W + j), p_fc));
}

std::vector<at::Tensor> dense_lstm_expand_fwd(
        at::Tensor xh, at::Tensor wl, at::Tensor bl, at::Tensor c_prev,
        at::Tensor pooled, at::Tensor table, at::Tensor ids,
        at::Tensor seed, at::Tensor expdrop, at::Tensor od_next,
        double fb, double p_lstm, double p_fc, int64_t s) {
    int64_t M = xh.size(0), N = wl.size(0);
    int B = c_prev.size(0), H = c_prev.size(1);
    int D = pooled.size(1), E = table.size(1);
    TORCH_CHECK(M == B && N == 4 * H);
    auto gates = at::empty({M, N}, xh.options());
    auto c_out = at::empty({B, H}, xh.options());
    auto sth_t = at::empty({B, H}, xh.options());
    hipStream_t stream = at::cuda::getCurrentCUDAStream();
    auto yf = skinny_slabs(stream, xh, wl);
    const bf16* bias_ptr = nullptr;
    if (bl.defined() && bl.numel() > 0)
        bias_ptr = (const bf16*)bl.data_ptr();
    bf16* od_ptr = nullptr;
    if (od_next.defined() && od_next.numel() > 0)
        od_ptr = (bf16*)od_next.data_ptr();
    int64_t n = (int64_t)B * (H + D + E);
    hipLaunchKernelGGL(skinny_epi_lstm_expand_kernel,
                       dim3(cdiv(n, 256)), dim3(256), 0, stream,
                       (const float*)yf.data_ptr(), bias_ptr,
                       (const bf16*)c_prev.data_ptr(),
                       (const bf16*)pooled.data_ptr(),
                       (const bf16*)table.data_ptr(),
                       (const int64_t*)ids.data_ptr(),
                       (const int64_t*)seed.data_ptr(),
                       (bf16*)gates.data_ptr(),
                       (bf16*)c_out.data_ptr(),
                       (bf16*)sth_t.data_ptr(),
                       (bf16*)expdrop.data_ptr(), od_ptr,
                       B, H, D, E, (int)yf.size(0),
                       (float)fb, (float)p_lstm, (float)p_fc, (int)s);
    HIP_OK(hipGetLastError());
    return {gates, c_out, sth_t};
}
```

sat_amd/ops/csrc/kernels.hip:

```cpp

#include "common.h"


__global__ void lstm_pw_fwd_kernel(const bf16* __restrict__ gates,
                                   const bf16* __restrict__ c,
                                   bf16* __restrict__ h_out,
                                   bf16* __restrict__ c_out,
                                   int B, int H, float fb) {
    int idx = blockIdx.x * blockDim.x + threadIdx.x;
    if (idx >= B * H) return;
    int b = idx / H, hh = idx % H;
    const bf16* gp = gates + (int64_t)b * 4 * H + hh;
    float g[4];
#pragma unroll
    for (int q = 0; q < 4; ++q) g[q] = bf2f(gp[q * H]);
    float cn, h;
    lstm_cell_fwd(g, bf2f(c[idx]), fb, cn, h);
    h_out[idx] = f2bf(h);
    c_out[idx] = f2bf(cn);
}

__global__ void lstm_pw_bwd_kernel(const bf16* __restrict__ gates,
                                   const bf16* __restrict__ c,
                                   const bf16* __restrict__ dh,
                                   const bf16* __restrict__ dc,
                                   bf16* __restrict__ dgates,
                                   bf16* __restrict__ dc_prev,
                                   int B, int H, float fb) {
    int idx = blockIdx.x * blockDim.x + threadIdx.x;
    if (idx >= B * H) return;
    int b = idx / H, hh = idx % H;
    const bf16* gp = gates + (int64_t)b * 4 * H + hh;
    float g[4], dg[4], dcp;
#pragma unroll
    for (int q = 0; q < 4; ++q) g[q] = bf2f(gp[q * H]);
    float dcv = (dc != nullptr) ? bf2f(dc[idx]) : 0.f;
    lstm_cell_bwd(g, bf2f(c[idx]), bf2f(dh[idx]), dcv, fb, dg, dcp);
    bf16* dgp = dgates + (int64_t)b * 4 * H + hh;
#pragma unroll
    for (int q = 0; q < 4; ++q) dgp[q * H] = f2bf(dg[q]);
    dc_prev[idx] = f2bf(dcp);
}

std::vector<at::Tensor> lstm_pointwise_fwd(at::Tensor gates, at::Tensor c,
                                           double fb) {
    CHECK_GPU(gates); CHECK_CONTIG(gates); CHECK_BF16(gates);
    CHECK_GPU(c); CHECK_CONTIG(c); CHECK_BF16(c);
    int B = c.size(0), H = c.size(1);
    TORCH_CHECK(gates.size(0) == B && gates.size(1) == 4 * H);
    auto h_out = at::empty_like(c);
    auto c_out = at::empty_like(c);
    int n = B * H;
    hipStream_t s = at::cuda::getCurrentCUDAStream();
    hipLaunchKernelGGL(lstm_pw_fwd_kernel, dim3(cdiv(n, 256)), dim3(256), 0, s,
                       (const bf16*)gates.data_ptr(), (const bf16*)c.data_ptr(),
                       (bf16*)h_out.data_ptr(), (bf16*)c_out.data_ptr(),
                       B, H, (float)fb);
    HIP_OK(hipGetLastError());
    return {h_out, c_out};
}

std::vector<at::Tensor> lstm_pointwise_bwd_out(at::Tensor gates,
                                               at::Tensor c, at::Tensor dh,
                                               at::Tensor dc, double fb,
                                               at::Tensor dgates_out) {
    CHECK_GPU(gates); CHECK_CONTIG(gates); CHECK_BF16(gates);
    int B = c.size(0), H = c.size(1);
    at::Tensor dgates;
    if (dgates_out.defined() && dgates_out.numel() > 0)
        dgates = dgates_out;
    else
        dgates = at::empty_like(gates);
    auto dc_prev = at::empty_like(c);
    const bf16* dc_ptr = nullptr;
    if (dc.defined() && dc.numel() > 0) dc_ptr = (const bf16*)dc.data_ptr();
    int n = B * H;
    hipStream_t s = at::cuda::getCurrentCUDAStream();
    hipLaunchKernelGGL(lstm_pw_bwd_kernel, dim3(cdiv(n, 256)), dim3(256), 0, s,
                       (const bf16*)gates.data_ptr(), (const bf16*)c.data_ptr(),
                       (const bf16*)dh.data_ptr(), dc_ptr,
                       (bf16*)dgates.data_ptr(), (bf16*)dc_prev.data_ptr(),
                       B, H, (float)fb);
    HIP_OK(hipGetLastError());
    return {dgates, dc_prev};
}

std::vector<at::Tensor> lstm_pointwise_bwd(at::Tensor gates, at::Tensor c,
                                           at::Tensor dh, at::Tensor dc,
                                           double fb) {
    return lstm_pointwise_bwd_out(gates, c, dh, dc, fb, at::Tensor());
}


__global__ void act_bwd_kernel(const bf16* __restrict__ dy,
                               const bf16* __restrict__ y,
                               bf16* __restrict__ dpre,
                               int64_t n, int act) {
    int64_t idx = (int64_t)blockIdx.x * blockDim.x + threadIdx.x;
    if (idx >= n) return;
    float g = bf2f(dy[idx]);
    float yv = bf2f(y[idx]);
    if (act == 1) g *= (1.f - yv * yv);
    else if (act == 2) g *= (yv > 0.f ? 1.f : 0.f);
    dpre[idx] = f2bf(g);
}

at::Tensor act_bwd(at::Tensor dy, at::Tensor y, int64_t act) {
    CHECK_GPU(dy); CHECK_CONTIG(dy); CHECK_BF16(dy);
    CHECK_GPU(y); CHECK_CONTIG(y); CHECK_BF16(y);
    auto dpre = at::empty_like(dy);
    int64_t n = dy.numel();
    hipStream_t s = at::cuda::getCurrentCUDAStream();
    hipLaunchKernelGGL(act_bwd_kernel, dim3(cdiv(n, 256)), dim3(256), 0, s,
                       (const bf16*)dy.data_ptr(), (const bf16*)y.data_ptr(),
                       (bf16*)dpre.data_ptr(), n, (int)act);
    HIP_OK(hipGetLastError());
    return dpre;
}


#define MAX_L 1024


__global__ void hash_dropout_kernel(const bf16* __restrict__ x,
                                    const int64_t* __restrict__ seed_p,
                                    bf16* __restrict__ y,
                                    int64_t n, float p, int salt) {
    const uint32_t seed = (uint32_t)(*seed_p);
    int64_t idx = (int64_t)blockIdx.x * blockDim.x + threadIdx.x;
    int64_t stride = (int64_t)gridDim.x * blockDim.x;
    for (int64_t i = idx * 8; i < n; i += stride * 8) {
        if (i + 8 <= n) {
            bf16x8 v = *(const bf16x8*)(x + i);
            bf16x8 o;
#pragma unroll
            for (int e = 0; e < 8; ++e)
                o[e] = f2bf(bf2f(v[e]) *
                            drop_scale(seed, salt, (uint32_t)(i + e), p));
            *(bf16x8*)(y + i) = o;
        } else {
            for (int64_t j = i; j < n; ++j)
                y[j] = f2bf(bf2f(x[j]) *
                            drop_scale(seed, salt, (uint32_t)j, p));
        }
    }
}

at::Tensor hash_dropout(at::Tensor x, at::Tensor seed, double p,
                        int64_t salt) {
    CHECK_GPU(x); CHECK_CONTIG(x); CHECK_BF16(x);
    if (p <= 0.0) return x;
    auto y = at::empty_like(x);
    int64_t n = x.numel();
    int blocks = (int)std::min<int64_t>(cdiv(n, 256 * 8), 4096);
    hipStream_t s = at::cuda::getCurrentCUDAStream();
    hipLaunchKernelGGL(hash_dropout_kernel, dim3(blocks), dim3(256), 0, s,
                       (const bf16*)x.data_ptr(),
                       (const int64_t*)seed.data_ptr(),
                       (bf16*)y.data_ptr(), n, (float)p, (int)salt);
    HIP_OK(hipGetLastError());
    return y;
}


__global__ void attn_scores_fused_kernel(
        const bf16* __restrict__ t1, const bf16* __restrict__ t2,
        const bf16* __restrict__ v, const int64_t* __restrict__ seed_p,
        bf16* __restrict__ tdrop, float* __restrict__ logits,
        int B, int L, int A, float p, int salt) {
    const uint32_t seed = (uint32_t)(*seed_p);
    int row = blockIdx.x * 4 + (threadIdx.x >> 6);
    if (row >= B * L) return;
    int lane = threadIdx.x & 63;
    int b = row / L;
    const bf16* t1r = t1 + (int64_t)row * A;
    const bf16* t2r = t2 + (int64_t)b * A;
    bf16* tdr = tdrop + (int64_t)row * A;
    float acc = 0.f;
    for (int a0 = lane * 8; a0 + 8 <= A; a0 += 64 * 8) {
        bf16x8 x1 = *(const bf16x8*)(t1r + a0);
        bf16x8 x2 = *(const bf16x8*)(t2r + a0);
        bf16x8 vv = *(const bf16x8*)(v + a0);
        bf16x8 out;
        float sc[8];
        drop_scale8(seed, salt, (uint32_t)((row * A + a0) >> 3), p, sc);
#pragma unroll
        for (int e = 0; e < 8; ++e) {
            float t = (bf2f(x1[e]) + bf2f(x2[e])) * sc[e];
            out[e] = f2bf(t);
            acc += t * bf2f(vv[e]);
        }
        *(bf16x8*)(tdr + a0) = out;
    }
    acc = wave_sum(acc);
    if (lane == 0) logits[row] = acc;
}

std::vector<at::Tensor> attn_scores_fused(at::Tensor t1, at::Tensor t2,
                                          at::Tensor v, at::Tensor seed,
                                          double p, int64_t salt,
                                          int64_t L) {
    CHECK_GPU(t1); CHECK_CONTIG(t1); CHECK_BF16(t1);
    CHECK_GPU(t2); CHECK_CONTIG(t2); CHECK_BF16(t2);
    CHECK_GPU(v); CHECK_CONTIG(v); CHECK_BF16(v);
    int A = t1.size(1);
    int rows = t1.size(0);
    int B = rows / (int)L;
    TORCH_CHECK(A % 8 == 0 && rows % L == 0);
    auto tdrop = at::empty_like(t1);
    auto logits = at::empty({B, (int)L},
                            t1.options().dtype(at::kFloat));
    hipStream_t s = at::cuda::getCurrentCUDAStream();
    hipLaunchKernelGGL(attn_scores_fused_kernel, dim3(cdiv(rows, 4)),
                       dim3(256), 0, s,
                       (const bf16*)t1.data_ptr(),
                       (const bf16*)t2.data_ptr(),
                       (const bf16*)v.data_ptr(),
                       (const int64_t*)seed.data_ptr(),
                       (bf16*)tdrop.data_ptr(), (float*)logits.data_ptr(),
                       B, (int)L, A, (float)p, (int)salt);
    HIP_OK(hipGetLastError());
    return {tdrop, logits};
}


__global__ void attn_pool_bwd_p1_kernel(
        const bf16* __restrict__ ctx, const float* __restrict__ alpha,
        const bf16* __restrict__ dpooled,
        float* __restrict__ sbuf, bf16* __restrict__ dctx,
        int L, int D) {
    int b = blockIdx.x;
    int nchunk = gridDim.y;
    int lchunk = (L + nchunk - 1) / nchunk;
    int l0 = blockIdx.y * lchunk;
    int l1 = min(L, l0 + lchunk);
    int wid = threadIdx.x >> 6, lane = threadIdx.x & 63;
    const bf16* cb = ctx + (int64_t)b * L * D;
    const bf16* dp = dpooled + (int64_t)b * D;

    for (int l = l0 + wid; l < l1; l += 4) {
        float acc = 0.f;
        float a = alpha[(int64_t)b * L + l];
        for (int d0 = lane * 8; d0 + 8 <= D; d0 += 64 * 8) {
            bf16x8 cv = *(const bf16x8*)(cb + (int64_t)l * D + d0);
            bf16x8 dv = *(const bf16x8*)(dp + d0);
            if (dctx != nullptr) {
                bf16x8 out;
#pragma unroll
                for (int e = 0; e < 8; ++e) {
                    float dpe = bf2f(dv[e]);
                    acc += bf2f(cv[e]) * dpe;
                    out[e] = f2bf(a * dpe);
                }
                *(bf16x8*)(dctx + (int64_t)b * L * D + (int64_t)l * D + d0)
                    = out;
            } else {
#pragma unroll
                for (int e = 0; e < 8; ++e)
                    acc += bf2f(cv[e]) * bf2f(dv[e]);
            }
        }
        acc = wave_sum(acc);
        if (lane == 0) sbuf[(int64_t)b * L + l] = acc;
    }
}

__global__ void attn_pool_bwd_p2_kernel(
        const float* __restrict__ alpha, const float* __restrict__ dalpha,
        const float* __restrict__ sbuf, float* __restrict__ dlogits,
        int L) {
    __shared__ float red[4];
    int b = blockIdx.x;
    int tid = threadIdx.x;
    float part = 0.f;
    for (int l = tid; l < L; l += blockDim.x) {
        float da = sbuf[(int64_t)b * L + l];
        if (dalpha != nullptr) da += dalpha[(int64_t)b * L + l];
        part += alpha[(int64_t)b * L + l] * da;
    }
    part = wave_sum(part);
    if ((tid & 63) == 0) red[tid >> 6] = part;
    __syncthreads();
    float dot = red[0] + red[1] + red[2] + red[3];
    for (int l = tid; l < L; l += blockDim.x) {
        float da = sbuf[(int64_t)b * L + l];
        if (dalpha != nullptr) da += dalpha[(int64_t)b * L + l];
        dlogits[(int64_t)b * L + l] =
            alpha[(int64_t)b * L + l] * (da - dot);
    }
}

__global__ void attn_pool_bwd_fused_kernel(
        const bf16* __restrict__ ctx, const float* __restrict__ alpha,
        const float* __restrict__ dalpha,
        const bf16* __restrict__ dpooled, bf16* __restrict__ dctx,
        float* __restrict__ dlogits, int L, int D) {
    __shared__ float sL[MAX_L];
    __shared__ float red[4];
    int b = blockIdx.x;
    int tid = threadIdx.x;
    int wid = tid >> 6, lane = tid & 63;
    const bf16* cb = ctx + (int64_t)b * L * D;
    const bf16* dp = dpooled + (int64_t)b * D;

    for (int l = wid; l < L; l += 4) {
        float acc = 0.f;
        float a = alpha[(int64_t)b * L + l];
        for (int d0 = lane * 8; d0 + 8 <= D; d0 += 64 * 8) {
            bf16x8 cv = *(const bf16x8*)(cb + (int64_t)l * D + d0);
            bf16x8 dv = *(const bf16x8*)(dp + d0);
            if (dctx != nullptr) {
                bf16x8 out;
#pragma unroll
                for (int e = 0; e < 8; ++e) {
                    float dpe = bf2f(dv[e]);
                    acc += bf2f(cv[e]) * dpe;
                    out[e] = f2bf(a * dpe);
                }
                *(bf16x8*)(dctx + (int64_t)b * L * D + (int64_t)l * D
                           + d0) = out;
            } else {
#pragma unroll
                for (int e = 0; e < 8; ++e)
                    acc += bf2f(cv[e]) * bf2f(dv[e]);
            }
        }
        acc = wave_sum(acc);
        if (lane == 0) sL[l] = acc;
    }
    __syncthreads();

    float part = 0.f;
    for (int l = tid; l < L; l += blockDim.x) {
        float da = sL[l];
        if (dalpha != nullptr) da += dalpha[(int64_t)b * L + l];
        part += alpha[(int64_t)b * L + l] * da;
    }
    part = wave_sum(part);
    if ((tid & 63) == 0) red[tid >> 6] = part;
    __syncthreads();
    float dot = red[0] + red[1] + red[2] + red[3];
    for (int l = tid; l < L; l += blockDim.x) {
        float da = sL[l];
        if (dalpha != nullptr) da += dalpha[(int64_t)b * L + l];
        dlogits[(int64_t)b * L + l] =
            alpha[(int64_t)b * L + l] * (da - dot);
    }
}

std::vector<at::Tensor> attn_pool_bwd(at::Tensor ctx, at::Tensor alpha,
                                      at::Tensor dalpha, at::Tensor dpooled,
                                      bool need_dctx) {
    CHECK_GPU(ctx); CHECK_CONTIG(ctx); CHECK_BF16(ctx);
    CHECK_GPU(alpha); CHECK_CONTIG(alpha); CHECK_F32(alpha);
    int B = ctx.size(0), L = ctx.size(1), D = ctx.size(2);
    TORCH_CHECK(L <= MAX_L && D % 8 == 0);
    auto dlogits = at::empty({B, L}, alpha.options());
    auto sbuf = at::empty({B, L}, alpha.options());
    at::Tensor dctx;
    bf16* dctx_ptr = nullptr;
    if (need_dctx) {
        dctx = at::empty_like(ctx);
        dctx_ptr = (bf16*)dctx.data_ptr();
    } else {
        dctx = at::empty({0}, ctx.options());
    }
    const float* dalpha_ptr = nullptr;
    if (dalpha.defined() && dalpha.numel() > 0)
        dalpha_ptr = (const float*)dalpha.data_ptr();
    hipStream_t s = at::cuda::getCurrentCUDAStream();
    hipLaunchKernelGGL(attn_pool_bwd_p1_kernel, dim3(B, 8), dim3(256), 0, s,
                       (const bf16*)ctx.data_ptr(),
                       (const float*)alpha.data_ptr(),
                       (const bf16*)dpooled.data_ptr(),
                       (float*)sbuf.data_ptr(), dctx_ptr, L, D);
    hipLaunchKernelGGL(attn_pool_bwd_p2_kernel, dim3(B), dim3(256), 0, s,
                       (const float*)alpha.data_ptr(), dalpha_ptr,
                       (const float*)sbuf.data_ptr(),
                       (float*)dlogits.data_ptr(), L);
    HIP_OK(hipGetLastError());
    return {dlogits, dctx};
}


template <int NCH>
__global__ void attn_scores_bwd_kernel(
        const bf16* __restrict__ tdrop, const bf16* __restrict__ v,
        const float* __restrict__ dlogits,
        const int64_t* __restrict__ seed_p,
        bf16* __restrict__ dt1, float* __restrict__ dt2,
        float* __restrict__ dvf,
        const bf16* __restrict__ t1y,
        int B, int L, int A, int lchunk, float p, int salt) {
    __shared__ float sdv[4][NCH * 512];
    __shared__ float sd2[4][NCH * 512];
    const uint32_t seed = (uint32_t)(*seed_p);
    int nchunk = (L + lchunk - 1) / lchunk;
    int b = blockIdx.x / nchunk;
    int l0 = (blockIdx.x % nchunk) * lchunk;
    int l1 = min(L, l0 + lchunk);
    int wid = threadIdx.x >> 6, lane = threadIdx.x & 63;

    float dv_acc[NCH][8] = {};
    float dt2_acc[NCH][8] = {};

    for (int l = l0 + wid; l < l1; l += 4) {
        int64_t row = (int64_t)b * L + l;
        float dl = dlogits[row];
#pragma unroll
        for (int ch = 0; ch < NCH; ++ch) {
            int a0 = ch * 512 + lane * 8;
            bf16x8 td = *(const bf16x8*)(tdrop + row * A + a0);
            bf16x8 vv = *(const bf16x8*)(v + a0);
            bf16x8 o;
            float sc[8];
            drop_scale8(seed, salt, (uint32_t)((row * A + a0) >> 3), p, sc);
            bf16x8 yv = {};
            if (t1y != nullptr)
                yv = *(const bf16x8*)(t1y + row * A + a0);
#pragma unroll
            for (int e = 0; e < 8; ++e) {
                dv_acc[ch][e] += bf2f(td[e]) * dl;
                float dt = dl * bf2f(vv[e]) * sc[e];
                dt2_acc[ch][e] += dt;
                if (t1y != nullptr) {
                    float y = bf2f(yv[e]);
                    dt *= (1.f - y * y);
                }
                o[e] = f2bf(dt);
            }
            *(bf16x8*)(dt1 + row * A + a0) = o;
        }
    }
#pragma unroll
    for (int ch = 0; ch < NCH; ++ch) {
        int a0 = ch * 512 + lane * 8;
#pragma unroll
        for (int e = 0; e < 8; ++e) {
            sdv[wid][a0 + e] = dv_acc[ch][e];
            sd2[wid][a0 + e] = dt2_acc[ch][e];
        }
    }
    __syncthreads();
    for (int a = threadIdx.x; a < A; a += (int)blockDim.x) {
        float dv_s = sdv[0][a] + sdv[1][a] + sdv[2][a] + sdv[3][a];
        float d2_s = sd2[0][a] + sd2[1][a] + sd2[2][a] + sd2[3][a];
        atomicAdd(dvf + a, dv_s);
        atomicAdd(dt2 + (int64_t)b * A + a, d2_s);
    }
}

std::vector<at::Tensor> attn_scores_bwd_tanh(
        at::Tensor tdrop, at::Tensor v, at::Tensor dlogits,
        at::Tensor seed, double p, int64_t salt, int64_t L,
        at::Tensor dv_acc, at::Tensor t1y, at::Tensor dt1_out);

std::vector<at::Tensor> attn_scores_bwd_acc(at::Tensor tdrop, at::Tensor v,
                                            at::Tensor dlogits,
                                            at::Tensor seed, double p,
                                            int64_t salt, int64_t L,
                                            at::Tensor dv_acc) {
    return attn_scores_bwd_tanh(tdrop, v, dlogits, seed, p, salt, L,
                                dv_acc, at::Tensor(), at::Tensor());
}

std::vector<at::Tensor> attn_scores_bwd_tanh(
        at::Tensor tdrop, at::Tensor v, at::Tensor dlogits,
        at::Tensor seed, double p, int64_t salt, int64_t L,
        at::Tensor dv_acc, at::Tensor t1y, at::Tensor dt1_out) {
    CHECK_GPU(tdrop); CHECK_CONTIG(tdrop); CHECK_BF16(tdrop);
    int rows = tdrop.size(0), A = tdrop.size(1);
    TORCH_CHECK(A % 512 == 0 && A <= 2048,
                "attn_scores_bwd requires A % 512 == 0, A <= 2048");
    int B = rows / (int)L;
    at::Tensor dt1;
    if (dt1_out.defined() && dt1_out.numel() > 0) {
        TORCH_CHECK(dt1_out.numel() == tdrop.numel());
        dt1 = dt1_out;
    } else {
        dt1 = at::empty_like(tdrop);
    }
    const bf16* t1y_ptr = nullptr;
    if (t1y.defined() && t1y.numel() > 0) {
        TORCH_CHECK(t1y.numel() == tdrop.numel());
        t1y_ptr = (const bf16*)t1y.data_ptr();
    }
    auto dt2 = at::zeros({B, A}, tdrop.options().dtype(at::kFloat));
    at::Tensor dvf;
    if (dv_acc.defined() && dv_acc.numel() > 0)
        dvf = dv_acc;
    else
        dvf = at::zeros({A}, tdrop.options().dtype(at::kFloat));
    int lchunk = ((int)L + 7) / 8;
    int nchunk = ((int)L + lchunk - 1) / lchunk;
    hipStream_t s = at::cuda::getCurrentCUDAStream();
#define LAUNCH_SB(NCH) \
    hipLaunchKernelGGL((attn_scores_bwd_kernel<NCH>), dim3(B * nchunk), \
                       dim3(256), 0, s, \
                       (const bf16*)tdrop.data_ptr(), \
                       (const bf16*)v.data_ptr(), \
                       (const float*)dlogits.data_ptr(), \
                       (const int64_t*)seed.data_ptr(), \
                       (bf16*)dt1.data_ptr(), (float*)dt2.data_ptr(), \
                       (float*)dvf.data_ptr(), t1y_ptr, \
                       B, (int)L, A, lchunk, (float)p, (int)salt)
    switch (A / 512) {
        case 1: LAUNCH_SB(1); break;
        case 2: LAUNCH_SB(2); break;
        case 3: LAUNCH_SB(3); break;
        default: LAUNCH_SB(4); break;
    }
#undef LAUNCH_SB
    HIP_OK(hipGetLastError());
    return {dt1, dt2, dvf};
}

std::vector<at::Tensor> attn_scores_bwd(at::Tensor tdrop, at::Tensor v,
                                        at::Tensor dlogits, at::Tensor seed,
                                        double p, int64_t salt, int64_t L) {
    return attn_scores_bwd_acc(tdrop, v, dlogits, seed, p, salt, L,
                               at::Tensor());
}

__global__ void attn_softmax_kernel(const float* __restrict__ logits,
                                    float* __restrict__ alpha, int L) {
    __shared__ float sa[MAX_L];
    __shared__ float red[8];
    int b = blockIdx.x;
    int tid = threadIdx.x;
    float lmax = -1e30f;
    for (int l = tid; l < L; l += blockDim.x) {
        float x = logits[(int64_t)b * L + l];
        sa[l] = x;
        lmax = fmaxf(lmax, x);
    }
    lmax = wave_max(lmax);
    if ((tid & 63) == 0) red[tid >> 6] = lmax;
    __syncthreads();
    float m = -1e30f;
    for (int w = 0; w < (int)(blockDim.x >> 6); ++w) m = fmaxf(m, red[w]);
    __syncthreads();
    float lsum = 0.f;
    for (int l = tid; l < L; l += blockDim.x) {
        float e = __expf(sa[l] - m);
        sa[l] = e;
        lsum += e;
    }
    lsum = wave_sum(lsum);
    if ((tid & 63) == 0) red[tid >> 6] = lsum;
    __syncthreads();
    float z = 0.f;
    for (int w = 0; w < (int)(blockDim.x >> 6); ++w) z += red[w];
    float inv = 1.0f / z;
    for (int l = tid; l < L; l += blockDim.x)
        alpha[(int64_t)b * L + l] = sa[l] * inv;
}

__global__ void attn_pool_sum_kernel(const bf16* __restrict__ ctx,
                                     const float* __restrict__ alpha,
                                     bf16* __restrict__ pooled,
                                     int L, int D) {
    __shared__ float sa[MAX_L];
    __shared__ float part[16][128 + 4];
    int b = blockIdx.x;
    int d0 = blockIdx.y * 128;
    int tid = threadIdx.x;
    for (int l = tid; l < L; l += blockDim.x)
        sa[l] = alpha[(int64_t)b * L + l];
    __syncthreads();
    int dg = tid & 15;
    int lg = tid >> 4;
    int d = d0 + dg * 8;
    float acc[8] = {};
    if (d < D) {
        const bf16* cb = ctx + (int64_t)b * L * D;
        for (int l = lg; l < L; l += 16) {
            bf16x8 cv = *(const bf16x8*)(cb + (int64_t)l * D + d);
            float a = sa[l];
#pragma unroll
            for (int e = 0; e < 8; ++e) acc[e] += a * bf2f(cv[e]);
        }
    }
#pragma unroll
    for (int e = 0; e < 8; ++e) part[lg][dg * 8 + e] = acc[e];
    __syncthreads();
    if (tid < 128 && d0 + tid < D) {
        float s = 0.f;
#pragma unroll
        for (int g = 0; g < 16; ++g) s += part[g][tid];
        pooled[(int64_t)b * D + d0 + tid] = f2bf(s);
    }
}

__global__ void attn_pool_fused_kernel(const bf16* __restrict__ ctx,
                                       const float* __restrict__ logits,
                                       float* __restrict__ alpha,
                                       bf16* __restrict__ pooled,
                                       int L, int D) {
    __shared__ float sa[MAX_L];
    __shared__ float red[8];
    __shared__ float part[16][128 + 4];
    int b = blockIdx.x;
    int d0 = blockIdx.y * 128;
    int tid = threadIdx.x;

    float lmax = -1e30f;
    for (int l = tid; l < L; l += blockDim.x) {
        float x = logits[(int64_t)b * L + l];
        sa[l] = x;
        lmax = fmaxf(lmax, x);
    }
    lmax = wave_max(lmax);
    if ((tid & 63) == 0) red[tid >> 6] = lmax;
    __syncthreads();
    float m = -1e30f;
    for (int w = 0; w < (int)(blockDim.x >> 6); ++w)
        m = fmaxf(m, red[w]);
    __syncthreads();
    float lsum = 0.f;
    for (int l = tid; l < L; l += blockDim.x) {
        float e = __expf(sa[l] - m);
        sa[l] = e;
        lsum += e;
    }
    lsum = wave_sum(lsum);
    if ((tid & 63) == 0) red[tid >> 6] = lsum;
    __syncthreads();
    float z = 0.f;
    for (int w = 0; w < (int)(blockDim.x >> 6); ++w) z += red[w];
    float inv = 1.0f / z;
    __syncthreads();
    for (int l = tid; l < L; l += blockDim.x) {
        sa[l] *= inv;
        if (blockIdx.y == 0)
            alpha[(int64_t)b * L + l] = sa[l];
    }
    __syncthreads();

    int dg = tid & 15;
    int lg = tid >> 4;
    int d = d0 + dg * 8;
    float acc[8] = {};
    if (d < D) {
        const bf16* cb = ctx + (int64_t)b * L * D;
        for (int l = lg; l < L; l += 16) {
            bf16x8 cv = *(const bf16x8*)(cb + (int64_t)l * D + d);
            float a = sa[l];
#pragma unroll
            for (int e = 0; e < 8; ++e) acc[e] += a * bf2f(cv[e]);
        }
    }
#pragma unroll
    for (int e = 0; e < 8; ++e) part[lg][dg * 8 + e] = acc[e];
    __syncthreads();
    if (tid < 128 && d0 + tid < D) {
        float ssum = 0.f;
#pragma unroll
        for (int g = 0; g < 16; ++g) ssum += part[g][tid];
        pooled[(int64_t)b * D + d0 + tid] = f2bf(ssum);
    }
}

std::vector<at::Tensor> attn_pool_fwd(at::Tensor ctx, at::Tensor logits) {
    CHECK_GPU(ctx); CHECK_CONTIG(ctx); CHECK_BF16(ctx);
    CHECK_GPU(logits); CHECK_CONTIG(logits); CHECK_F32(logits);
    int B = ctx.size(0), L = ctx.size(1), D = ctx.size(2);
    TORCH_CHECK(L <= MAX_L, "attention locations exceed LDS stage");
    auto alpha = at::empty({B, L}, ctx.options().dtype(at::kFloat));
    auto pooled = at::empty({B, D}, ctx.options());
    hipStream_t s = at::cuda::getCurrentCUDAStream();
    hipLaunchKernelGGL(attn_pool_fused_kernel, dim3(B, cdiv(D, 128)),
                       dim3(256), 0, s,
                       (const bf16*)ctx.data_ptr(),
                       (const float*)logits.data_ptr(),
                       (float*)alpha.data_ptr(),
                       (bf16*)pooled.data_ptr(), L, D);
    HIP_OK(hipGetLastError());
    return {alpha, pooled};
}


__global__ void embedding_fwd_kernel(const int64_t* __restrict__ ids,
                                     const bf16* __restrict__ table,
                                     bf16* __restrict__ out,
                                     int B, int E) {
    int idx = blockIdx.x * blockDim.x + threadIdx.x;
    if (idx >= B * E) return;
    int b = idx / E, e = idx % E;
    out[idx] = table[ids[b] * E + e];
}

__global__ void embedding_bwd_kernel(const int64_t* __restrict__ ids,
                                     const bf16* __restrict__ dy,
                                     float* __restrict__ dtable,
                                     int B, int E) {
    int idx = blockIdx.x * blockDim.x + threadIdx.x;
    if (idx >= B * E) return;
    int b = idx / E, e = idx % E;
    atomicAdd(dtable + ids[b] * E + e, bf2f(dy[idx]));
}

at::Tensor embedding_fwd(at::Tensor ids, at::Tensor table) {
    CHECK_GPU(ids); CHECK_CONTIG(ids);
    CHECK_GPU(table); CHECK_CONTIG(table); CHECK_BF16(table);
    TORCH_CHECK(ids.scalar_type() == at::kLong, "ids must be int64");
    int B = ids.numel(), E = table.size(1);
    auto out = at::empty({B, E}, table.options());
    hipStream_t s = at::cuda::getCurrentCUDAStream();
    hipLaunchKernelGGL(embedding_fwd_kernel, dim3(cdiv(B * E, 256)),
                       dim3(256), 0, s,
                       (const int64_t*)ids.data_ptr(),
                       (const bf16*)table.data_ptr(),
                       (bf16*)out.data_ptr(), B, E);
    HIP_OK(hipGetLastError());
    return out;
}

at::Tensor embedding_bwd(at::Tensor ids, at::Tensor dy, int64_t rows) {
    CHECK_GPU(ids); CHECK_GPU(dy); CHECK_CONTIG(dy); CHECK_BF16(dy);
    int B = ids.numel(), E = dy.size(1);
    auto dtable = at::zeros({rows, E}, dy.options().dtype(at::kFloat));
    hipStream_t s = at::cuda::getCurrentCUDAStream();
    hipLaunchKernelGGL(embedding_bwd_kernel, dim3(cdiv(B * E, 256)),
                       dim3(256), 0, s,
                       (const int64_t*)ids.data_ptr(),
                       (const bf16*)dy.data_ptr(),
                       (float*)dtable.data_ptr(), B, E);
    HIP_OK(hipGetLastError());
    return dtable;
}


__global__ void ce_fwd_kernel(const bf16* __restrict__ logits,
                              const int64_t* __restrict__ labels,
                              const float* __restrict__ mask,
                              float* __restrict__ losses,
                              float* __restrict__ lse,
                              int V) {
    __shared__ float red[8];
    int b = blockIdx.x;
    int tid = threadIdx.x;
    const bf16* row = logits + (int64_t)b * V;

    float lmax = -1e30f;
    for (int v = tid; v < V; v += blockDim.x)
        lmax = fmaxf(lmax, bf2f(row[v]));
    lmax = wave_max(lmax);
    if ((tid & 63) == 0) red[tid >> 6] = lmax;
    __syncthreads();
    float m = -1e30f;
    for (int w = 0; w < (int)(blockDim.x >> 6); ++w) m = fmaxf(m, red[w]);
    __syncthreads();

    float lsum = 0.f;
    for (int v = tid; v < V; v += blockDim.x)
        lsum += __expf(bf2f(row[v]) - m);
    lsum = wave_sum(lsum);
    if ((tid & 63) == 0) red[tid >> 6] = lsum;
    __syncthreads();
    if (tid == 0) {
        float z = 0.f;
        for (int w = 0; w < (int)(blockDim.x >> 6); ++w) z += red[w];
        float l = m + __logf(z);
        lse[b] = l;
        losses[b] = (l - bf2f(row[labels[b]])) * mask[b];
    }
}

__global__ void ce_bwd_kernel(const bf16* __restrict__ logits,
                              const int64_t* __restrict__ labels,
                              const float* __restrict__ mask,
                              const float* __restrict__ lse,
                              const float* __restrict__ dloss,
                              bf16* __restrict__ dlogits,
                              int B, int V) {
    int64_t idx = (int64_t)blockIdx.x * blockDim.x + threadIdx.x;
    if (idx >= (int64_t)B * V) return;
    int b = idx / V, v = idx % V;
    float p = __expf(bf2f(logits[idx]) - lse[b]);
    float g = (p - (labels[b] == v ? 1.f : 0.f)) * mask[b] * dloss[b];
    dlogits[idx] = f2bf(g);
}

std::vector<at::Tensor> ce_fwd(at::Tensor logits, at::Tensor labels,
                               at::Tensor mask) {
    CHECK_GPU(logits); CHECK_CONTIG(logits); CHECK_BF16(logits);
    CHECK_GPU(labels); CHECK_GPU(mask); CHECK_F32(mask);
    int B = logits.size(0), V = logits.size(1);
    auto losses = at::empty({B}, logits.options().dtype(at::kFloat));
    auto lse = at::empty({B}, logits.options().dtype(at::kFloat));
    hipStream_t s = at::cuda::getCurrentCUDAStream();
    hipLaunchKernelGGL(ce_fwd_kernel, dim3(B), dim3(256), 0, s,
                       (const bf16*)logits.data_ptr(),
                       (const int64_t*)labels.data_ptr(),
                       (const float*)mask.data_ptr(),
                       (float*)losses.data_ptr(), (float*)lse.data_ptr(), V);
    HIP_OK(hipGetLastError());
    return {losses, lse};
}

at::Tensor ce_bwd(at::Tensor logits, at::Tensor labels, at::Tensor mask,
                  at::Tensor lse, at::Tensor dloss) {
    CHECK_GPU(logits); CHECK_CONTIG(logits); CHECK_BF16(logits);
    int B = logits.size(0), V = logits.size(1);
    auto dlogits = at::empty_like(logits);
    hipStream_t s = at::cuda::getCurrentCUDAStream();
    hipLaunchKernelGGL(ce_bwd_kernel,
                       dim3(cdiv((int64_t)B * V, 256)), dim3(256), 0, s,
                       (const bf16*)logits.data_ptr(),
                       (const int64_t*)labels.data_ptr(),
                       (const float*)mask.data_ptr(),
                       (const float*)lse.data_ptr(),
                       (const float*)dloss.data_ptr(),
                       (bf16*)dlogits.data_ptr(), B, V);
    HIP_OK(hipGetLastError());
    return dlogits;
}


__global__ void sq_norm_kernel(const float* __restrict__ g, int64_t n,
                               float* __restrict__ out) {
    int64_t idx = (int64_t)blockIdx.x * blockDim.x + threadIdx.x;
    float acc = 0.f;
    for (int64_t i = idx; i < n; i += (int64_t)gridDim.x * blockDim.x)
        acc += g[i] * g[i];
    acc = wave_sum(acc);
    __shared__ float red[8];
    if ((threadIdx.x & 63) == 0) red[threadIdx.x >> 6] = acc;
    __syncthreads();
    if (threadIdx.x == 0) {
        float t = 0.f;
        for (int w = 0; w < (int)(blockDim.x >> 6); ++w) t += red[w];
        atomicAdd(out, t);
    }
}

__global__ void adam_kernel(float* __restrict__ p, const float* __restrict__ g,
                            float* __restrict__ m, float* __restrict__ v,
                            const float* __restrict__ gsq,
                            const float* __restrict__ step_dev,
                            int64_t n, float lr0, float decay_factor,
                            float steps_per_decay, float b1, float b2,
                            float eps, float clip) {
    float step = *step_dev;
    float bc1 = 1.f - powf(b1, step);
    float bc2 = 1.f - powf(b2, step);
    float lr = lr0;
    if (decay_factor < 1.f)
        lr = lr0 * powf(decay_factor, floorf(step / steps_per_decay));
    float scale = 1.f;
    if (clip > 0.f) {
        float norm = sqrtf(*gsq);
        if (norm > clip) scale = clip / norm;
    }
    int64_t idx = (int64_t)blockIdx.x * blockDim.x + threadIdx.x;
    for (int64_t i = idx; i < n; i += (int64_t)gridDim.x * blockDim.x) {
        float gi = g[i] * scale;
        float mi = b1 * m[i] + (1.f - b1) * gi;
        float vi = b2 * v[i] + (1.f - b2) * gi * gi;
        m[i] = mi;
        v[i] = vi;
        float mhat = mi / bc1;
        float vhat = vi / bc2;
        p[i] -= lr * mhat / (sqrtf(vhat) + eps);
    }
}

at::Tensor grad_sq_norm(std::vector<at::Tensor> grads) {
    TORCH_CHECK(!grads.empty());
    auto out = at::zeros({1}, grads[0].options().dtype(at::kFloat));
    hipStream_t s = at::cuda::getCurrentCUDAStream();
    for (auto& g : grads) {
        CHECK_GPU(g); CHECK_CONTIG(g); CHECK_F32(g);
        int64_t n = g.numel();
        int blocks = (int)std::min<int64_t>(cdiv(n, 256), 1024);
        hipLaunchKernelGGL(sq_norm_kernel, dim3(blocks), dim3(256), 0, s,
                           (const float*)g.data_ptr(), n,
                           (float*)out.data_ptr());
    }
    HIP_OK(hipGetLastError());
    return out;
}

void adam_step(std::vector<at::Tensor> params, std::vector<at::Tensor> grads,
               std::vector<at::Tensor> ms, std::vector<at::Tensor> vs,
               at::Tensor step_dev, double lr0, double decay_factor,
               double steps_per_decay, double b1, double b2, double eps,
               double clip, at::Tensor gsq) {
    CHECK_GPU(step_dev); CHECK_F32(step_dev);
    hipStream_t s = at::cuda::getCurrentCUDAStream();
    for (size_t i = 0; i < params.size(); ++i) {
        auto& p = params[i];
        CHECK_GPU(p); CHECK_CONTIG(p); CHECK_F32(p);
        int64_t n = p.numel();
        int blocks = (int)std::min<int64_t>(cdiv(n, 256), 2048);
        hipLaunchKernelGGL(adam_kernel, dim3(blocks), dim3(256), 0, s,
                           (float*)p.data_ptr(),
                           (const float*)grads[i].data_ptr(),
                           (float*)ms[i].data_ptr(), (float*)vs[i].data_ptr(),
                           (const float*)gsq.data_ptr(),
                           (const float*)step_dev.data_ptr(), n,
                           (float)lr0, (float)decay_factor,
                           (float)steps_per_decay, (float)b1, (float)b2,
                           (float)eps, (float)clip);
    }
    HIP_OK(hipGetLastError());
}


__global__ void sq_norm_mt_kernel(const int64_t* __restrict__ desc,
                                  const int64_t* __restrict__ cum,
                                  int n_tensors, int64_t total,
                                  float* __restrict__ out) {
    extern __shared__ int64_t scum[];
    for (int i = threadIdx.x; i <= n_tensors; i += blockDim.x)
        scum[i] = cum[i];
    __syncthreads();
    float acc = 0.f;
    int64_t idx = (int64_t)blockIdx.x * blockDim.x + threadIdx.x;
    int64_t stride = (int64_t)gridDim.x * blockDim.x;
    for (int64_t i = idx; i < total; i += stride) {
        int lo = 0, hi = n_tensors;
        while (hi - lo > 1) {
            int mid = (lo + hi) >> 1;
            if (i >= scum[mid]) lo = mid; else hi = mid;
        }
        const float* g = (const float*)desc[lo * 5 + 1];
        float gv = g[i - scum[lo]];
        acc += gv * gv;
    }
    acc = wave_sum(acc);
    __shared__ float red[4];
    if ((threadIdx.x & 63) == 0) red[threadIdx.x >> 6] = acc;
    __syncthreads();
    if (threadIdx.x == 0)
        atomicAdd(out, red[0] + red[1] + red[2] + red[3]);
}

at::Tensor sq_norm_mt(at::Tensor desc, at::Tensor cum, int64_t n_tensors,
                      int64_t total) {
    auto out = at::zeros({1}, at::TensorOptions()
                                  .dtype(at::kFloat)
                                  .device(desc.device()));
    hipStream_t s = at::cuda::getCurrentCUDAStream();
    int blocks = (int)std::min<int64_t>(cdiv(total, 256 * 8), 2048);
    size_t shm = (n_tensors + 1) * sizeof(int64_t);
    hipLaunchKernelGGL(sq_norm_mt_kernel, dim3(blocks), dim3(256), shm, s,
                       (const int64_t*)desc.data_ptr(),
                       (const int64_t*)cum.data_ptr(),
                       (int)n_tensors, total, (float*)out.data_ptr());
    HIP_OK(hipGetLastError());
    return out;
}

typedef __attribute__((ext_vector_type(4))) float floatx4v;

template <int VEC4>
__global__ void adam_mt_kernel(const int64_t* __restrict__ desc,
                               const int64_t* __restrict__ cum,
                               int n_tensors, int64_t total,
                               const float* __restrict__ gsq,
                               const float* __restrict__ step_dev,
                               float lr0, float decay_factor,
                               float steps_per_decay, float b1, float b2,
                               float eps, float clip, int zero_g) {
    extern __shared__ int64_t scum[];
    for (int i = threadIdx.x; i <= n_tensors; i += blockDim.x)
        scum[i] = cum[i];
    __syncthreads();
    float step = *step_dev;
    float bc1 = 1.f - powf(b1, step);
    float bc2 = 1.f - powf(b2, step);
    float lr = lr0;
    if (decay_factor < 1.f)
        lr = lr0 * powf(decay_factor, floorf(step / steps_per_decay));
    float scale = 1.f;
    if (clip > 0.f) {
        float norm = sqrtf(*gsq);
        if (norm > clip) scale = clip / norm;
    }
    constexpr int V = VEC4 ? 4 : 1;
    int64_t idx = (int64_t)blockIdx.x * blockDim.x + threadIdx.x;
    int64_t stride = (int64_t)gridDim.x * blockDim.x;
    int64_t niter = (total + V - 1) / V;
    for (int64_t it = idx; it < niter; it += stride) {
        int64_t i = it * V;
        int lo = 0, hi = n_tensors;
        while (hi - lo > 1) {
            int mid = (lo + hi) >> 1;
            if (i >= scum[mid]) lo = mid; else hi = mid;
        }
        int64_t off = i - scum[lo];
        float* p = (float*)desc[lo * 5 + 0];
        float* g = (float*)desc[lo * 5 + 1];
        float* m = (float*)desc[lo * 5 + 2];
        float* v = (float*)desc[lo * 5 + 3];
        bf16* sh = (bf16*)desc[lo * 5 + 4];
        if (VEC4) {
            floatx4v g4 = *(floatx4v*)(g + off);
            floatx4v m4 = *(floatx4v*)(m + off);
            floatx4v v4 = *(floatx4v*)(v + off);
            floatx4v p4 = *(floatx4v*)(p + off);
#pragma unroll
            for (int e = 0; e < 4; ++e) {
                float gi = g4[e] * scale;
                float mi = b1 * m4[e] + (1.f - b1) * gi;
                float vi = b2 * v4[e] + (1.f - b2) * gi * gi;
                m4[e] = mi;
                v4[e] = vi;
                p4[e] -= lr * (mi / bc1) / (sqrtf(vi / bc2) + eps);
            }
            *(floatx4v*)(m + off) = m4;
            *(floatx4v*)(v + off) = v4;
            *(floatx4v*)(p + off) = p4;
            if (sh != nullptr) {
#pragma unroll
                for (int e = 0; e < 4; ++e)
                    sh[off + e] = f2bf(p4[e]);
            }
            if (zero_g)
                *(floatx4v*)(g + off) = floatx4v{0.f, 0.f, 0.f, 0.f};
        } else {
            float gi = g[off] * scale;
            float mi = b1 * m[off] + (1.f - b1) * gi;
            float vi = b2 * v[off] + (1.f - b2) * gi * gi;
            m[off] = mi;
            v[off] = vi;
            float pn = p[off]
                - lr * (mi / bc1) / (sqrtf(vi / bc2) + eps);
            p[off] = pn;
            if (sh != nullptr) sh[off] = f2bf(pn);
            if (zero_g) g[off] = 0.f;
        }
    }
}

void adam_step_mt(at::Tensor desc, at::Tensor cum, int64_t n_tensors,
                  int64_t total, at::Tensor step_dev, double lr0,
                  double decay_factor, double steps_per_decay, double b1,
                  double b2, double eps, double clip, at::Tensor gsq,
                  bool zero_grads, bool vec4) {
    hipStream_t s = at::cuda::getCurrentCUDAStream();
    int blocks = (int)std::min<int64_t>(cdiv(total, 256 * 4), 4096);
    size_t shm = (n_tensors + 1) * sizeof(int64_t);
    if (vec4)
        hipLaunchKernelGGL((adam_mt_kernel<1>), dim3(blocks), dim3(256),
                           shm, s,
                           (const int64_t*)desc.data_ptr(),
                           (const int64_t*)cum.data_ptr(),
                           (int)n_tensors, total,
                           (const float*)gsq.data_ptr(),
                           (const float*)step_dev.data_ptr(),
                           (float)lr0, (float)decay_factor,
                           (float)steps_per_decay, (float)b1, (float)b2,
                           (float)eps, (float)clip, zero_grads ? 1 : 0);
    else
        hipLaunchKernelGGL((adam_mt_kernel<0>), dim3(blocks), dim3(256),
                           shm, s,
                           (const int64_t*)desc.data_ptr(),
                           (const int64_t*)cum.data_ptr(),
                           (int)n_tensors, total,
                           (const float*)gsq.data_ptr(),
                           (const float*)step_dev.data_ptr(),
                           (float)lr0, (float)decay_factor,
                           (float)steps_per_decay, (float)b1, (float)b2,
                           (float)eps, (float)clip, zero_grads ? 1 : 0);
    HIP_OK(hipGetLastError());
}
```

Baseline: 5768 images/sec.

## Chain per-step decoder kernels to drop LSTM-input and tanh-backward launches

Result: faster. 5896 images/sec, median of 6 (+2.2%).

```diff
diff --git a/sat_amd/models/bptt.py b/sat_amd/models/bptt.py
--- a/sat_amd/models/bptt.py
+++ b/sat_amd/models/bptt.py
@@ -4,6 +4,8 @@
 from sat_amd import _C
 
 ACT_NONE, ACT_TANH, ACT_RELU = 0, 1, 2
+
+CHAIN_FUSION = True
 
 
 def _drop(x, seed, p, salt):
@@ -61,8 +63,12 @@
         empty_b = _EMPTY_B(dev)
         fuse_small = (B <= 128 and (I + H) % 32 == 0
                       and (H + D + E) % 32 == 0)
+        chain = fuse_small and CHAIN_FUSION
 
         _C.hash_dropout_out(init_output, seed, p_fc, 1, ODROP[0:B])
+        if chain:
+            _C.lstm_in_tail(emb_c, last_word, state_h, seed, p_lstm, 3,
+                            XH[0:B], D)
 
         for t in range(T):
             s = t * 16
@@ -73,13 +79,23 @@
             t2 = _C.dense_fwd(ODROP[sl], w1b_c, b1b_c, ACT_TANH)
             tdrop, att_logits = _C.attn_scores_fused(
                 t1, t2, v_c, seed, p_fc, s + 2, L)
-            alpha, pooled = _C.attn_pool_fwd(contexts, att_logits)
-
-            _C.lstm_in_fuse(pooled, emb_c, last_word, state_h, seed,
-                            p_lstm, s + 3, XH[sl])
+            if chain:
+                alpha, pooled = _C.attn_pool_fwd_xh(
+                    contexts, att_logits, seed, p_lstm, s + 3, XH[sl], I)
+            else:
+                alpha, pooled = _C.attn_pool_fwd(contexts, att_logits)
+                _C.lstm_in_fuse(pooled, emb_c, last_word, state_h, seed,
+                                p_lstm, s + 3, XH[sl])
             od_next = ODROP[(t + 1) * B:(t + 2) * B] if t + 1 < T \
                 else empty_b
-            if fuse_small:
+            if chain:
+                xh_next = XH[(t + 1) * B:(t + 2) * B] if t + 1 < T \
+                    else empty_b
+                gates, c_new, sth_t = _C.dense_lstm_expand_xh_fwd(
+                    XH[sl], wl_c, bl_c, memory, pooled, emb_c,
+                    last_word, seed, EXPD[sl], od_next,
+                    1.0, p_lstm, p_fc, s, labels_cat[sl], xh_next)
+            elif fuse_small:
                 gates, c_new, sth_t = _C.dense_lstm_expand_fwd(
                     XH[sl], wl_c, bl_c, memory, pooled, emb_c,
                     last_word, seed, EXPD[sl], od_next,
@@ -116,6 +132,7 @@
         ctx_ag.p_fc = p_fc
         ctx_ag.p_lstm = p_lstm
         ctx_ag.train_cnn = train_cnn
+        ctx_ag.chain = chain
         return EXPD, attn_acc
 
     @staticmethod
@@ -147,6 +164,11 @@
         dv_acc = torch.zeros_like(v, dtype=torch.float32)
         dctx_acc = torch.zeros_like(contexts) if need_dctx else None
 
+        chain = ctx_ag.chain
+        DT2 = torch.zeros(T, B, A, dtype=torch.float32, device=dev) \
+            if chain else None
+        carry_slabs, carry_salt = None, 0
+
         d_out_carry = torch.zeros(B, H, dtype=torch.bfloat16, device=dev)
         d_sth_carry = torch.zeros(B, H, dtype=torch.bfloat16, device=dev)
         dc_carry = torch.zeros(B, H, dtype=torch.bfloat16, device=dev)
@@ -154,10 +176,16 @@
         for t in range(T - 1, -1, -1):
             s = t * 16
             sl = slice(t * B, (t + 1) * B)
-            dc_prev, dpool_dec, demb_dec = _C.dexp_lstm_bwd(
-                d_expd[sl], d_out_carry, d_sth_carry, seed,
-                gates_l[t], cprev_l[t], dc_carry, DG[sl],
-                p_fc, p_lstm, s, D, E, 1.0)
+            if carry_slabs is not None:
+                dc_prev, dpool_dec, demb_dec = _C.dexp_lstm_bwd_slabs(
+                    d_expd[sl], carry_slabs, carry_salt, d_sth_carry,
+                    seed, gates_l[t], cprev_l[t], dc_carry, DG[sl],
+                    p_fc, p_lstm, s, D, E, 1.0)
+            else:
+                dc_prev, dpool_dec, demb_dec = _C.dexp_lstm_bwd(
+                    d_expd[sl], d_out_carry, d_sth_carry, seed,
+                    gates_l[t], cprev_l[t], dc_carry, DG[sl],
+                    p_fc, p_lstm, s, D, E, 1.0)
             dgates = DG[sl]
             if B <= 128:
                 dpooled, d_sth_carry = _C.dense_dx_fuse(
@@ -178,18 +206,32 @@
             if need_dctx:
                 dctx_acc += dctx_t
             sl_a = slice(t * B * L, (t + 1) * B * L)
-            _dt1, dt2f, _dv = _C.attn_scores_bwd_tanh(
-                tdrops[t], v, dlog_att, seed, p_fc, s + 2, L, dv_acc,
-                t1s[t], DPRE1A[sl_a])
-
-            _C.act_bwd_f32_out(dt2f, t2s[t], ACT_TANH, DPRE1B[sl])
-            d_out_carry = _C.dense_fwd_drop(DPRE1B[sl], w1b_t, seed,
-                                            p_fc, s + 1)
+            if chain:
+                _dt1, dt2f, _dv = _C.attn_scores_bwd_step(
+                    tdrops[t], v, dlog_att, seed, p_fc, s + 2, L, dv_acc,
+                    t1s[t], DPRE1A[sl_a], DT2[t])
+            else:
+                _dt1, dt2f, _dv = _C.attn_scores_bwd_tanh(
+                    tdrops[t], v, dlog_att, seed, p_fc, s + 2, L, dv_acc,
+                    t1s[t], DPRE1A[sl_a])
+
+            if chain:
+                carry_slabs = _C.dense_tanhbwd_slabs(dt2f, t2s[t], w1b_t,
+                                                     DPRE1B[sl])
+                carry_salt = s + 1
+            else:
+                _C.act_bwd_f32_out(dt2f, t2s[t], ACT_TANH, DPRE1B[sl])
+                d_out_carry = _C.dense_fwd_drop(DPRE1B[sl], w1b_t, seed,
+                                                p_fc, s + 1)
 
             if need_dctx:
                 dcd = DPRE1A[sl_a].matmul(w1a)
                 dctx_acc += _drop(dcd, seed, p_fc, s + 0) \
                     .reshape(B, L, D)
+
+        if carry_slabs is not None:
+            d_out_carry = _C.slab_epilogue_drop(carry_slabs, seed, p_fc,
+                                                carry_salt)
 
         if CDROP is not None:
             dW1a = torch.bmm(
diff --git a/sat_amd/ops/csrc/bindings.cpp b/sat_amd/ops/csrc/bindings.cpp
--- a/sat_amd/ops/csrc/bindings.cpp
+++ b/sat_amd/ops/csrc/bindings.cpp
@@ -128,6 +128,32 @@
                double steps_per_decay, double b1, double b2, double eps,
                double clip, at::Tensor gsq);
 
+std::vector<at::Tensor> attn_scores_bwd_step(
+    at::Tensor tdrop, at::Tensor v, at::Tensor dlogits, at::Tensor seed,
+    double p, int64_t salt, int64_t L, at::Tensor dv_acc, at::Tensor t1y,
+    at::Tensor dt1_out, at::Tensor dt2_out);
+std::vector<at::Tensor> attn_pool_fwd_xh(at::Tensor ctx, at::Tensor logits,
+                                         at::Tensor seed, double p,
+                                         int64_t salt, at::Tensor xh,
+                                         int64_t I);
+void lstm_in_tail(at::Tensor table, at::Tensor ids, at::Tensor sth,
+                  at::Tensor seed, double p, int64_t salt, at::Tensor xh,
+                  int64_t D);
+std::vector<at::Tensor> dense_lstm_expand_xh_fwd(
+    at::Tensor xh, at::Tensor wl, at::Tensor bl, at::Tensor c_prev,
+    at::Tensor pooled, at::Tensor table, at::Tensor ids, at::Tensor seed,
+    at::Tensor expdrop, at::Tensor od_next, double fb, double p_lstm,
+    double p_fc, int64_t s, at::Tensor next_ids, at::Tensor xh_next);
+at::Tensor dense_tanhbwd_slabs(at::Tensor dy, at::Tensor y, at::Tensor w,
+                               at::Tensor dpre_out);
+at::Tensor slab_epilogue_drop(at::Tensor yf, at::Tensor seed, double p,
+                              int64_t salt);
+std::vector<at::Tensor> dexp_lstm_bwd_slabs(
+    at::Tensor dexpd, at::Tensor carry_slabs, int64_t carry_salt,
+    at::Tensor d_sth_carry, at::Tensor seed, at::Tensor gates,
+    at::Tensor c_prev, at::Tensor dc, at::Tensor dgates_out, double p_fc,
+    double p_lstm, int64_t s, int64_t D, int64_t E, double fb);
+
 PYBIND11_MODULE(TORCH_EXTENSION_NAME, m) {
     m.def("dense_fwd", &dense_fwd, "MFMA GEMM + bias/act (bf16)");
     m.def("dense_fwd_drop", &dense_fwd_drop,
@@ -183,4 +209,21 @@
     m.def("sq_norm_mt", &sq_norm_mt);
     m.def("adam_step_mt", &adam_step_mt);
     m.def("adam_step", &adam_step);
+    m.def("attn_scores_bwd_step", &attn_scores_bwd_step,
+          "attn_scores_bwd_tanh into a caller-zeroed dt2 slice");
+    m.def("attn_pool_fwd_xh", &attn_pool_fwd_xh,
+          "attention pool that also writes the dropped pooled columns "
+          "of the LSTM input");
+    m.def("lstm_in_tail", &lstm_in_tail,
+          "embedding + state columns of the LSTM input (step 0)");
+    m.def("dense_lstm_expand_xh_fwd", &dense_lstm_expand_xh_fwd,
+          "dense_lstm_expand_fwd that also lays down the next step's "
+          "embedding + state LSTM-input columns");
+    m.def("dense_tanhbwd_slabs", &dense_tanhbwd_slabs,
+          "split-K slabs of (dy * (1 - y^2)) @ w^T, tanh backward built "
+          "in the A-operand load");
+    m.def("slab_epilogue_drop", &slab_epilogue_drop,
+          "bf16(sum of split-K slabs * dropout mask)");
+    m.def("dexp_lstm_bwd_slabs", &dexp_lstm_bwd_slabs,
+          "dexp_lstm_bwd taking d_out_carry as split-K slabs + salt");
 }
diff --git a/sat_amd/ops/csrc/bptt_fuse.hip b/sat_amd/ops/csrc/bptt_fuse.hip
--- a/sat_amd/ops/csrc/bptt_fuse.hip
+++ b/sat_amd/ops/csrc/bptt_fuse.hip
@@ -16,6 +16,7 @@
     int64_t idx = (int64_t)blockIdx.x * blockDim.x + threadIdx.x;
     if (idx >= (int64_t)B * W) return;
     int b = idx / W, j = idx % W;
+    if (j < D && pooled == nullptr) return;
     float val;
     if (j < I) {
         val = (j < D) ? bf2f(pooled[(int64_t)b * D + j])
@@ -42,6 +43,25 @@
                        (const bf16*)sth.data_ptr(),
                        (const int64_t*)seed.data_ptr(),
                        (bf16*)xh.data_ptr(), B, D, E, H,
+                       (float)p, (int)salt);
+    HIP_OK(hipGetLastError());
+}
+
+void lstm_in_tail(at::Tensor table, at::Tensor ids, at::Tensor sth,
+                  at::Tensor seed, double p, int64_t salt, at::Tensor xh,
+                  int64_t D) {
+    int B = sth.size(0), E = table.size(1), H = sth.size(1);
+    TORCH_CHECK(xh.is_contiguous() && xh.numel() == (int64_t)B * (D + E + H)
+                && ids.numel() == B);
+    int64_t n = (int64_t)B * (D + E + H);
+    hipStream_t s = at::cuda::getCurrentCUDAStream();
+    hipLaunchKernelGGL(lstm_in_fuse_kernel, dim3(cdiv(n, 256)), dim3(256),
+                       0, s, (const bf16*)nullptr,
+                       (const bf16*)table.data_ptr(),
+                       (const int64_t*)ids.data_ptr(),
+                       (const bf16*)sth.data_ptr(),
+                       (const int64_t*)seed.data_ptr(),
+                       (bf16*)xh.data_ptr(), B, (int)D, E, H,
                        (float)p, (int)salt);
     HIP_OK(hipGetLastError());
 }
@@ -390,7 +410,9 @@
                                      bf16* __restrict__ demb_dec,
                                      int B, int H, int D, int E,
                                      float p_fc, float p_lstm, int s,
-                                     float fb) {
+                                     float fb,
+                                     const float* __restrict__ carry_slabs,
+                                     int carry_splitk, int carry_salt) {
     const uint32_t seed = (uint32_t)(*seed_p);
     const int W = H + D + E;
     int64_t idx = (int64_t)blockIdx.x * blockDim.x + threadIdx.x;
@@ -400,7 +422,16 @@
         * drop_scale(seed, s + 6, (uint32_t)(b * W + j), p_fc);
     if (j < H) {
         uint32_t hidx = (uint32_t)(b * H + j);
-        float dout = dexp + bf2f(d_out_carry[(int64_t)b * H + j]);
+        float doc;
+        if (carry_slabs != nullptr) {
+            float v = sum_slabs(carry_slabs, (int64_t)B * H,
+                                (int64_t)b * H + j, carry_splitk);
+            v *= drop_scale(seed, carry_salt, hidx, p_fc);
+            doc = bf2f(f2bf(v));
+        } else {
+            doc = bf2f(d_out_carry[(int64_t)b * H + j]);
+        }
+        float dout = dexp + doc;
         float dhv = dout * drop_scale(seed, s + 4, hidx, p_lstm)
             + bf2f(d_sth_carry[(int64_t)b * H + j])
             * drop_scale(seed, s + 5, hidx, p_lstm);
@@ -422,17 +453,14 @@
     }
 }
 
-std::vector<at::Tensor> dexp_lstm_bwd(at::Tensor dexpd,
-                                      at::Tensor d_out_carry,
-                                      at::Tensor d_sth_carry,
-                                      at::Tensor seed, at::Tensor gates,
-                                      at::Tensor c_prev, at::Tensor dc,
-                                      at::Tensor dgates_out,
-                                      double p_fc, double p_lstm,
-                                      int64_t s, int64_t D, int64_t E,
-                                      double fb) {
+static std::vector<at::Tensor> dexp_lstm_bwd_impl(
+        at::Tensor dexpd, const bf16* carry_ptr, const float* slab_ptr,
+        int carry_splitk, int64_t carry_salt, at::Tensor d_sth_carry,
+        at::Tensor seed, at::Tensor gates, at::Tensor c_prev,
+        at::Tensor dc, at::Tensor dgates_out, double p_fc, double p_lstm,
+        int64_t s, int64_t D, int64_t E, double fb) {
     CHECK_GPU(dexpd); CHECK_BF16(dexpd);
-    int B = d_out_carry.size(0), H = d_out_carry.size(1);
+    int B = d_sth_carry.size(0), H = d_sth_carry.size(1);
     TORCH_CHECK(dexpd.numel() == (int64_t)B * (H + D + E));
     TORCH_CHECK(dgates_out.numel() == (int64_t)B * 4 * H);
     auto dc_prev = at::empty({B, H}, dexpd.options());
@@ -445,8 +473,7 @@
     hipStream_t st = at::cuda::getCurrentCUDAStream();
     hipLaunchKernelGGL(dexp_lstm_bwd_kernel, dim3(cdiv(n, 256)),
                        dim3(256), 0, st,
-                       (const bf16*)dexpd.data_ptr(),
-                       (const bf16*)d_out_carry.data_ptr(),
+                       (const bf16*)dexpd.data_ptr(), carry_ptr,
                        (const bf16*)d_sth_carry.data_ptr(),
                        (const int64_t*)seed.data_ptr(),
                        (const bf16*)gates.data_ptr(),
@@ -456,7 +483,49 @@
                        (bf16*)dpool_dec.data_ptr(),
                        (bf16*)demb_dec.data_ptr(),
                        B, H, (int)D, (int)E,
-                       (float)p_fc, (float)p_lstm, (int)s, (float)fb);
+                       (float)p_fc, (float)p_lstm, (int)s, (float)fb,
+                       slab_ptr, carry_splitk, (int)carry_salt);
     HIP_OK(hipGetLastError());
     return {dc_prev, dpool_dec, demb_dec};
 }
+
+std::vector<at::Tensor> dexp_lstm_bwd(at::Tensor dexpd,
+                                      at::Tensor d_out_carry,
+                                      at::Tensor d_sth_carry,
+                                      at::Tensor seed, at::Tensor gates,
+                                      at::Tensor c_prev, at::Tensor dc,
+                                      at::Tensor dgates_out,
+                                      double p_fc, double p_lstm,
+                                      int64_t s, int64_t D, int64_t E,
+                                      double fb) {
+    TORCH_CHECK(d_out_carry.numel() == d_sth_carry.numel());
+    return dexp_lstm_bwd_impl(dexpd, (const bf16*)d_out_carry.data_ptr(),
+                              nullptr, 0, 0, d_sth_carry, seed, gates,
+                              c_prev, dc, dgates_out, p_fc, p_lstm, s, D,
+                              E, fb);
+}
+
+std::vector<at::Tensor> dexp_lstm_bwd_slabs(at::Tensor dexpd,
+                                            at::Tensor carry_slabs,
+                                            int64_t carry_salt,
+                                            at::Tensor d_sth_carry,
+                                            at::Tensor seed,
+                                            at::Tensor gates,
+                                            at::Tensor c_prev,
+                                            at::Tensor dc,
+                                            at::Tensor dgates_out,
+                                            double p_fc, double p_lstm,
+                                            int64_t s, int64_t D,
+                                            int64_t E, double fb) {
+    CHECK_GPU(carry_slabs); CHECK_CONTIG(carry_slabs);
+    CHECK_F32(carry_slabs);
+    TORCH_CHECK(carry_slabs.dim() == 3
+                && carry_slabs.size(1) == d_sth_carry.size(0)
+                && carry_slabs.size(2) == d_sth_carry.size(1),
+                "carry slabs must be [splitk, B, H]");
+    return dexp_lstm_bwd_impl(dexpd, nullptr,
+                              (const float*)carry_slabs.data_ptr(),
+                              (int)carry_slabs.size(0), carry_salt,
+                              d_sth_carry, seed, gates, c_prev, dc,
+                              dgates_out, p_fc, p_lstm, s, D, E, fb);
+}
diff --git a/sat_amd/ops/csrc/gemm.hip b/sat_amd/ops/csrc/gemm.hip
--- a/sat_amd/ops/csrc/gemm.hip
+++ b/sat_amd/ops/csrc/gemm.hip
@@ -141,14 +141,17 @@
 }
 
 
-template <int RF>
+template <int RF, bool TANHA>
 __global__ __launch_bounds__(256)
 void skinny_gemm_kernel(const bf16* __restrict__ A,
                         const bf16* __restrict__ W,
                         const bf16* __restrict__ bias,
                         bf16* __restrict__ Y,
                         float* __restrict__ Yf,
-                        int M, int N, int K, int act, int splitk) {
+                        int M, int N, int K, int act, int splitk,
+                        const float* __restrict__ Af,
+                        const bf16* __restrict__ Ay,
+                        bf16* __restrict__ Apre) {
     const int lane = threadIdx.x & 63;
     const int wave = threadIdx.x >> 6;
     const int n0 = blockIdx.x * 64 + wave * 16;
@@ -186,6 +189,22 @@
             for (int mi = 0; mi < RF; ++mi) {
                 bf16x8 a0 = {};
                 int ar = mi * 16 + lrow;
+                if constexpr (TANHA) {
+                    if (ar < M) {
+                        const int64_t ao = (int64_t)ar * K + kof;
+                        floatx4 g0 = *(const floatx4*)(Af + ao);
+                        floatx4 g1 = *(const floatx4*)(Af + ao + 4);
+                        bf16x8 yv = *(const bf16x8*)(Ay + ao);
+#pragma unroll
+                        for (int e = 0; e < 8; ++e) {
+                            float y = bf2f(yv[e]);
+                            float g = e < 4 ? g0[e] : g1[e - 4];
+                            a0[e] = f2bf(g * (1.f - y * y));
+                        }
+                        if (blockIdx.x == 0 && wave == 0)
+                            *(bf16x8*)(Apre + ao) = a0;
+                    }
+                } else
                 if (kof + 8 <= K) {
                     if (ar < M)
                         a0 = *(const bf16x8*)(A + (int64_t)ar * K + kof);
@@ -267,13 +286,44 @@
     const int M = x.size(0), K = x.size(1), N = w.size(0);
     TORCH_CHECK(is_skinny(M, K),
                 "skinny GEMM: M <= 128 and K % 32 == 0 only");
-    auto kernel = M <= 32 ? skinny_gemm_kernel<2>
-                : M <= 64 ? skinny_gemm_kernel<4>
-                          : skinny_gemm_kernel<8>;
+    auto kernel = M <= 32 ? skinny_gemm_kernel<2, false>
+                : M <= 64 ? skinny_gemm_kernel<4, false>
+                          : skinny_gemm_kernel<8, false>;
     hipLaunchKernelGGL(kernel, dim3(plan.nblocks, plan.splitk), dim3(256),
                        0, stream, (const bf16*)x.data_ptr(),
                        (const bf16*)w.data_ptr(), bias, y, yf, M, N, K,
-                       act, plan.splitk);
+                       act, plan.splitk, (const float*)nullptr,
+                       (const bf16*)nullptr, (bf16*)nullptr);
+}
+
+at::Tensor dense_tanhbwd_slabs(at::Tensor dy, at::Tensor y, at::Tensor w,
+                               at::Tensor dpre_out) {
+    CHECK_GPU(dy); CHECK_CONTIG(dy); CHECK_F32(dy);
+    CHECK_GPU(y); CHECK_CONTIG(y); CHECK_BF16(y);
+    CHECK_GPU(w); CHECK_CONTIG(w); CHECK_BF16(w);
+    CHECK_GPU(dpre_out); CHECK_CONTIG(dpre_out); CHECK_BF16(dpre_out);
+    TORCH_CHECK(dy.dim() == 2 && w.dim() == 2);
+    const int M = dy.size(0), K = dy.size(1), N = w.size(0);
+    TORCH_CHECK(w.size(1) == K && y.numel() == dy.numel()
+                && dpre_out.numel() == dy.numel(), "shape mismatch");
+    TORCH_CHECK(is_skinny(M, K),
+                "skinny GEMM: M <= 128 and K % 32 == 0 only");
+    SkinnyPlan plan = skinny_plan(N, K);
+    auto yf = at::empty({plan.splitk, M, N}, dy.options());
+    auto kernel = M <= 32 ? skinny_gemm_kernel<2, true>
+                : M <= 64 ? skinny_gemm_kernel<4, true>
+                          : skinny_gemm_kernel<8, true>;
+    hipStream_t stream = at::cuda::getCurrentCUDAStream();
+    hipLaunchKernelGGL(kernel, dim3(plan.nblocks, plan.splitk), dim3(256),
+                       0, stream, (const bf16*)nullptr,
+                       (const bf16*)w.data_ptr(), (const bf16*)nullptr,
+                       (bf16*)nullptr, (float*)yf.data_ptr(), M, N, K,
+                       ACT_NONE, plan.splitk,
+                       (const float*)dy.data_ptr(),
+                       (const bf16*)y.data_ptr(),
+                       (bf16*)dpre_out.data_ptr());
+    HIP_OK(hipGetLastError());
+    return yf;
 }
 
 static at::Tensor skinny_slabs(hipStream_t stream, const at::Tensor& x,
@@ -397,6 +447,23 @@
     hipStream_t stream = at::cuda::getCurrentCUDAStream();
     auto yf = skinny_slabs(stream, x, w);
     int64_t n = M * N;
+    hipLaunchKernelGGL(skinny_epilogue_drop_kernel,
+                       dim3(cdiv(n, 256)), dim3(256), 0, stream,
+                       (const float*)yf.data_ptr(), (bf16*)y.data_ptr(),
+                       (const int64_t*)seed.data_ptr(), n,
+                       (int)yf.size(0), (float)p, (int)salt);
+    HIP_OK(hipGetLastError());
+    return y;
+}
+
+at::Tensor slab_epilogue_drop(at::Tensor yf, at::Tensor seed, double p,
+                              int64_t salt) {
+    CHECK_GPU(yf); CHECK_CONTIG(yf); CHECK_F32(yf);
+    TORCH_CHECK(yf.dim() == 3, "slabs must be [splitk, M, N]");
+    auto y = at::empty({yf.size(1), yf.size(2)},
+                       yf.options().dtype(at::kBFloat16));
+    int64_t n = y.numel();
+    hipStream_t stream = at::cuda::getCurrentCUDAStream();
     hipLaunchKernelGGL(skinny_epilogue_drop_kernel,
                        dim3(cdiv(n, 256)), dim3(256), 0, stream,
                        (const float*)yf.data_ptr(), (bf16*)y.data_ptr(),
@@ -644,9 +711,12 @@
         bf16* __restrict__ sth_t, bf16* __restrict__ expdrop,
         bf16* __restrict__ od_next,
         int B, int H, int D, int E, int splitk,
-        float fb, float p_lstm, float p_fc, int s) {
+        float fb, float p_lstm, float p_fc, int s,
+        const int64_t* __restrict__ next_ids,
+        bf16* __restrict__ xh_next) {
     const uint32_t seed = (uint32_t)(*seed_p);
     const int W = H + D + E;
+    const int I = D + E;
     int64_t idx = (int64_t)blockIdx.x * blockDim.x + threadIdx.x;
     if (idx >= (int64_t)B * W) return;
     int b = idx / W, j = idx % W;
@@ -658,8 +728,10 @@
         c_out[(int64_t)b * H + j] = f2bf(cn);
         uint32_t hidx = (uint32_t)(b * H + j);
         float ot = h * drop_scale(seed, s + 4, hidx, p_lstm);
-        sth_t[(int64_t)b * H + j] =
-            f2bf(h * drop_scale(seed, s + 5, hidx, p_lstm));
+        bf16 sth = f2bf(h * drop_scale(seed, s + 5, hidx, p_lstm));
+        sth_t[(int64_t)b * H + j] = sth;
+        if (xh_next != nullptr)
+            xh_next[(int64_t)b * W + I + j] = sth;
         if (od_next != nullptr)
             od_next[(int64_t)b * H + j] =
                 f2bf(ot * drop_scale(seed, s + 16 + 1, hidx, p_fc));
@@ -667,17 +739,24 @@
     } else if (j < H + D) {
         val = bf2f(pooled[(int64_t)b * D + (j - H)]);
     } else {
-        val = bf2f(table[ids[b] * E + (j - H - D)]);
+        int e = j - H - D;
+        val = bf2f(table[ids[b] * E + e]);
+        if (xh_next != nullptr)
+            xh_next[(int64_t)b * W + D + e] =
+                f2bf(bf2f(table[next_ids[b] * E + e])
+                     * drop_scale(seed, s + 16 + 3,
+                                  (uint32_t)(b * I + D + e), p_lstm));
     }
     expdrop[idx] = f2bf(val * drop_scale(seed, s + 6,
                                          (uint32_t)(b * W + j), p_fc));
 }
 
-std::vector<at::Tensor> dense_lstm_expand_fwd(
+static std::vector<at::Tensor> dense_lstm_expand_impl(
         at::Tensor xh, at::Tensor wl, at::Tensor bl, at::Tensor c_prev,
         at::Tensor pooled, at::Tensor table, at::Tensor ids,
         at::Tensor seed, at::Tensor expdrop, at::Tensor od_next,
-        double fb, double p_lstm, double p_fc, int64_t s) {
+        double fb, double p_lstm, double p_fc, int64_t s,
+        const int64_t* next_ids_ptr, bf16* xh_next_ptr) {
     int64_t M = xh.size(0), N = wl.size(0);
     int B = c_prev.size(0), H = c_prev.size(1);
     int D = pooled.size(1), E = table.size(1);
@@ -707,7 +786,41 @@
                        (bf16*)sth_t.data_ptr(),
                        (bf16*)expdrop.data_ptr(), od_ptr,
                        B, H, D, E, (int)yf.size(0),
-                       (float)fb, (float)p_lstm, (float)p_fc, (int)s);
+                       (float)fb, (float)p_lstm, (float)p_fc, (int)s,
+                       next_ids_ptr, xh_next_ptr);
     HIP_OK(hipGetLastError());
     return {gates, c_out, sth_t};
 }
+
+std::vector<at::Tensor> dense_lstm_expand_fwd(
+        at::Tensor xh, at::Tensor wl, at::Tensor bl, at::Tensor c_prev,
+        at::Tensor pooled, at::Tensor table, at::Tensor ids,
+        at::Tensor seed, at::Tensor expdrop, at::Tensor od_next,
+        double fb, double p_lstm, double p_fc, int64_t s) {
+    return dense_lstm_expand_impl(xh, wl, bl, c_prev, pooled, table, ids,
+                                  seed, expdrop, od_next, fb, p_lstm, p_fc,
+                                  s, nullptr, nullptr);
+}
+
+std::vector<at::Tensor> dense_lstm_expand_xh_fwd(
+        at::Tensor xh, at::Tensor wl, at::Tensor bl, at::Tensor c_prev,
+        at::Tensor pooled, at::Tensor table, at::Tensor ids,
+        at::Tensor seed, at::Tensor expdrop, at::Tensor od_next,
+        double fb, double p_lstm, double p_fc, int64_t s,
+        at::Tensor next_ids, at::Tensor xh_next) {
+    const int64_t* nid = nullptr;
+    bf16* xn = nullptr;
+    if (xh_next.defined() && xh_next.numel() > 0) {
+        CHECK_GPU(xh_next); CHECK_CONTIG(xh_next); CHECK_BF16(xh_next);
+        CHECK_GPU(next_ids); CHECK_CONTIG(next_ids);
+        TORCH_CHECK(next_ids.scalar_type() == at::kLong
+                    && next_ids.numel() == c_prev.size(0));
+        TORCH_CHECK(xh_next.numel() == c_prev.size(0)
+                    * (c_prev.size(1) + pooled.size(1) + table.size(1)));
+        nid = (const int64_t*)next_ids.data_ptr();
+        xn = (bf16*)xh_next.data_ptr();
+    }
+    return dense_lstm_expand_impl(xh, wl, bl, c_prev, pooled, table, ids,
+                                  seed, expdrop, od_next, fb, p_lstm, p_fc,
+                                  s, nid, xn);
+}
diff --git a/sat_amd/ops/csrc/kernels.hip b/sat_amd/ops/csrc/kernels.hip
--- a/sat_amd/ops/csrc/kernels.hip
+++ b/sat_amd/ops/csrc/kernels.hip
@@ -290,64 +290,6 @@
     }
 }
 
-__global__ void attn_pool_bwd_fused_kernel(
-        const bf16* __restrict__ ctx, const float* __restrict__ alpha,
-        const float* __restrict__ dalpha,
-        const bf16* __restrict__ dpooled, bf16* __restrict__ dctx,
-        float* __restrict__ dlogits, int L, int D) {
-    __shared__ float sL[MAX_L];
-    __shared__ float red[4];
-    int b = blockIdx.x;
-    int tid = threadIdx.x;
-    int wid = tid >> 6, lane = tid & 63;
-    const bf16* cb = ctx + (int64_t)b * L * D;
-    const bf16* dp = dpooled + (int64_t)b * D;
-
-    for (int l = wid; l < L; l += 4) {
-        float acc = 0.f;
-        float a = alpha[(int64_t)b * L + l];
-        for (int d0 = lane * 8; d0 + 8 <= D; d0 += 64 * 8) {
-            bf16x8 cv = *(const bf16x8*)(cb + (int64_t)l * D + d0);
-            bf16x8 dv = *(const bf16x8*)(dp + d0);
-            if (dctx != nullptr) {
-                bf16x8 out;
-#pragma unroll
-                for (int e = 0; e < 8; ++e) {
-                    float dpe = bf2f(dv[e]);
-                    acc += bf2f(cv[e]) * dpe;
-                    out[e] = f2bf(a * dpe);
-                }
-                *(bf16x8*)(dctx + (int64_t)b * L * D + (int64_t)l * D
-                           + d0) = out;
-            } else {
-#pragma unroll
-                for (int e = 0; e < 8; ++e)
-                    acc += bf2f(cv[e]) * bf2f(dv[e]);
-            }
-        }
-        acc = wave_sum(acc);
-        if (lane == 0) sL[l] = acc;
-    }
-    __syncthreads();
-
-    float part = 0.f;
-    for (int l = tid; l < L; l += blockDim.x) {
-        float da = sL[l];
-        if (dalpha != nullptr) da += dalpha[(int64_t)b * L + l];
-        part += alpha[(int64_t)b * L + l] * da;
-    }
-    part = wave_sum(part);
-    if ((tid & 63) == 0) red[tid >> 6] = part;
-    __syncthreads();
-    float dot = red[0] + red[1] + red[2] + red[3];
-    for (int l = tid; l < L; l += blockDim.x) {
-        float da = sL[l];
-        if (dalpha != nullptr) da += dalpha[(int64_t)b * L + l];
-        dlogits[(int64_t)b * L + l] =
-            alpha[(int64_t)b * L + l] * (da - dot);
-    }
-}
-
 std::vector<at::Tensor> attn_pool_bwd(at::Tensor ctx, at::Tensor alpha,
                                       at::Tensor dalpha, at::Tensor dpooled,
                                       bool need_dctx) {
@@ -450,24 +392,11 @@
     }
 }
 
-std::vector<at::Tensor> attn_scores_bwd_tanh(
+static std::vector<at::Tensor> attn_scores_bwd_impl(
         at::Tensor tdrop, at::Tensor v, at::Tensor dlogits,
         at::Tensor seed, double p, int64_t salt, int64_t L,
-        at::Tensor dv_acc, at::Tensor t1y, at::Tensor dt1_out);
-
-std::vector<at::Tensor> attn_scores_bwd_acc(at::Tensor tdrop, at::Tensor v,
-                                            at::Tensor dlogits,
-                                            at::Tensor seed, double p,
-                                            int64_t salt, int64_t L,
-                                            at::Tensor dv_acc) {
-    return attn_scores_bwd_tanh(tdrop, v, dlogits, seed, p, salt, L,
-                                dv_acc, at::Tensor(), at::Tensor());
-}
-
-std::vector<at::Tensor> attn_scores_bwd_tanh(
-        at::Tensor tdrop, at::Tensor v, at::Tensor dlogits,
-        at::Tensor seed, double p, int64_t salt, int64_t L,
-        at::Tensor dv_acc, at::Tensor t1y, at::Tensor dt1_out) {
+        at::Tensor dv_acc, at::Tensor t1y, at::Tensor dt1_out,
+        at::Tensor dt2_out) {
     CHECK_GPU(tdrop); CHECK_CONTIG(tdrop); CHECK_BF16(tdrop);
     int rows = tdrop.size(0), A = tdrop.size(1);
     TORCH_CHECK(A % 512 == 0 && A <= 2048,
@@ -485,7 +414,14 @@
         TORCH_CHECK(t1y.numel() == tdrop.numel());
         t1y_ptr = (const bf16*)t1y.data_ptr();
     }
-    auto dt2 = at::zeros({B, A}, tdrop.options().dtype(at::kFloat));
+    at::Tensor dt2;
+    if (dt2_out.defined() && dt2_out.numel() > 0) {
+        CHECK_GPU(dt2_out); CHECK_CONTIG(dt2_out); CHECK_F32(dt2_out);
+        TORCH_CHECK(dt2_out.numel() == (int64_t)B * A);
+        dt2 = dt2_out;
+    } else {
+        dt2 = at::zeros({B, A}, tdrop.options().dtype(at::kFloat));
+    }
     at::Tensor dvf;
     if (dv_acc.defined() && dv_acc.numel() > 0)
         dvf = dv_acc;
@@ -515,6 +451,32 @@
     return {dt1, dt2, dvf};
 }
 
+std::vector<at::Tensor> attn_scores_bwd_tanh(
+        at::Tensor tdrop, at::Tensor v, at::Tensor dlogits,
+        at::Tensor seed, double p, int64_t salt, int64_t L,
+        at::Tensor dv_acc, at::Tensor t1y, at::Tensor dt1_out) {
+    return attn_scores_bwd_impl(tdrop, v, dlogits, seed, p, salt, L,
+                                dv_acc, t1y, dt1_out, at::Tensor());
+}
+
+std::vector<at::Tensor> attn_scores_bwd_acc(at::Tensor tdrop, at::Tensor v,
+                                            at::Tensor dlogits,
+                                            at::Tensor seed, double p,
+                                            int64_t salt, int64_t L,
+                                            at::Tensor dv_acc) {
+    return attn_scores_bwd_tanh(tdrop, v, dlogits, seed, p, salt, L,
+                                dv_acc, at::Tensor(), at::Tensor());
+}
+
+std::vector<at::Tensor> attn_scores_bwd_step(
+        at::Tensor tdrop, at::Tensor v, at::Tensor dlogits,
+        at::Tensor seed, double p, int64_t salt, int64_t L,
+        at::Tensor dv_acc, at::Tensor t1y, at::Tensor dt1_out,
+        at::Tensor dt2_out) {
+    return attn_scores_bwd_impl(tdrop, v, dlogits, seed, p, salt, L,
+                                dv_acc, t1y, dt1_out, dt2_out);
+}
+
 std::vector<at::Tensor> attn_scores_bwd(at::Tensor tdrop, at::Tensor v,
                                         at::Tensor dlogits, at::Tensor seed,
                                         double p, int64_t salt, int64_t L) {
@@ -596,7 +558,11 @@
                                        const float* __restrict__ logits,
                                        float* __restrict__ alpha,
                                        bf16* __restrict__ pooled,
-                                       int L, int D) {
+                                       int L, int D,
+                                       bf16* __restrict__ xh,
+                                       const int64_t* __restrict__ seed_p,
+                                       int xh_stride, int I, float p,
+                                       int salt) {
     __shared__ float sa[MAX_L];
     __shared__ float red[8];
     __shared__ float part[16][128 + 4];
@@ -657,15 +623,26 @@
         float ssum = 0.f;
 #pragma unroll
         for (int g = 0; g < 16; ++g) ssum += part[g][tid];
-        pooled[(int64_t)b * D + d0 + tid] = f2bf(ssum);
-    }
-}
-
-std::vector<at::Tensor> attn_pool_fwd(at::Tensor ctx, at::Tensor logits) {
+        bf16 pv = f2bf(ssum);
+        pooled[(int64_t)b * D + d0 + tid] = pv;
+        if (xh != nullptr) {
+            int d = d0 + tid;
+            xh[(int64_t)b * xh_stride + d] =
+                f2bf(bf2f(pv) * drop_scale((uint32_t)(*seed_p), salt,
+                                           (uint32_t)(b * I + d), p));
+        }
+    }
+}
+
+static std::vector<at::Tensor> attn_pool_fwd_impl(
+        at::Tensor ctx, at::Tensor logits, bf16* xh_ptr,
+        const int64_t* seed_ptr, int xh_stride, int I, double p,
+        int64_t salt) {
     CHECK_GPU(ctx); CHECK_CONTIG(ctx); CHECK_BF16(ctx);
     CHECK_GPU(logits); CHECK_CONTIG(logits); CHECK_F32(logits);
     int B = ctx.size(0), L = ctx.size(1), D = ctx.size(2);
     TORCH_CHECK(L <= MAX_L, "attention locations exceed LDS stage");
+    TORCH_CHECK(logits.numel() == (int64_t)B * L);
     auto alpha = at::empty({B, L}, ctx.options().dtype(at::kFloat));
     auto pooled = at::empty({B, D}, ctx.options());
     hipStream_t s = at::cuda::getCurrentCUDAStream();
@@ -674,9 +651,29 @@
                        (const bf16*)ctx.data_ptr(),
                        (const float*)logits.data_ptr(),
                        (float*)alpha.data_ptr(),
-                       (bf16*)pooled.data_ptr(), L, D);
+                       (bf16*)pooled.data_ptr(), L, D,
+                       xh_ptr, seed_ptr, xh_stride, I, (float)p,
+                       (int)salt);
     HIP_OK(hipGetLastError());
     return {alpha, pooled};
+}
+
+std::vector<at::Tensor> attn_pool_fwd(at::Tensor ctx, at::Tensor logits) {
+    return attn_pool_fwd_impl(ctx, logits, nullptr, nullptr, 0, 0, 0.0, 0);
+}
+
+std::vector<at::Tensor> attn_pool_fwd_xh(at::Tensor ctx, at::Tensor logits,
+                                         at::Tensor seed, double p,
+                                         int64_t salt, at::Tensor xh,
+                                         int64_t I) {
+    CHECK_GPU(xh); CHECK_CONTIG(xh); CHECK_BF16(xh);
+    CHECK_GPU(seed);
+    TORCH_CHECK(xh.dim() == 2 && xh.size(0) == ctx.size(0)
+                && I >= ctx.size(2) && xh.size(1) >= I,
+                "xh must be [B, I + H] with I >= D");
+    return attn_pool_fwd_impl(ctx, logits, (bf16*)xh.data_ptr(),
+                              (const int64_t*)seed.data_ptr(),
+                              (int)xh.size(1), (int)I, p, salt);
 }
 
 
```
